# igloo-io/igloo

Hardware: AMD Instinct MI355X
Metric: TPC-H SF100 total query time (s) + rows/sec scan, 1/2/4/8 MI355X (lower is better)
Workload: dtype exact decimal(15,2) int64 fixed-point / int32 keys

## Files before the change

csrc/bindings.cpp:

```cpp
#include <pybind11/pybind11.h>
#include <pybind11/stl.h>

#include <tuple>
#include <memory>
#include <vector>

#include "io/parquet_meta.h"
#include "kernels/kernels.h"
#include "runtime/runtime.h"
#include "sql/ast.h"
#include "sql/ast_py.h"

namespace py = pybind11;
using namespace igloo;

namespace {

template <typename T>
T* P(uintptr_t p) {
  return reinterpret_cast<T*>(p);
}
hipStream_t S(uintptr_t s) { return reinterpret_cast<hipStream_t>(s); }

template <typename T>
struct py_arg {
  using type = T;
  static T get(T v) { return v; }
};
template <typename T>
struct py_arg<T*> {
  using type = uintptr_t;
  static T* get(uintptr_t v) { return reinterpret_cast<T*>(v); }
};
template <auto F>
struct raw_t;
template <typename R, typename... A, R (*F)(A...)>
struct raw_t<F> {
  R operator()(typename py_arg<A>::type... a) const { return F(py_arg<A>::get(a)...); }
};
template <auto F>
constexpr raw_t<F> raw{};

using AggDescArg = std::vector<std::tuple<int, int, uintptr_t, uintptr_t, uintptr_t, uintptr_t>>;
std::vector<kern::AggDesc> agg_descs(const AggDescArg& descs) {
  std::vector<kern::AggDesc> d;
  for (auto& t : descs)
    d.push_back({std::get<0>(t), std::get<1>(t), P<const void>(std::get<2>(t)), P<const uint8_t>(std::get<3>(t)),
                 P<void>(std::get<4>(t)), P<void>(std::get<5>(t))});
  return d;
}

py::list parse(const std::string& text) {
  py::list out;
  try {
    for (auto& st : sql::parse_sql(text)) out.append(sql::to_python(st));
  } catch (const sql::ParseError& e) {
    PyErr_SetString(PyExc_SyntaxError, e.what());
    throw py::error_already_set();
  }
  return out;
}

py::list tokenize(const std::string& text) {
  py::list out;
  static const char* names[] = {"ident", "quoted_ident", "keyword", "number", "string", "op", "end"};
  try {
    for (auto& t : sql::tokenize(text)) out.append(py::make_tuple(names[t.kind], t.text, t.pos));
  } catch (const sql::ParseError& e) {
    PyErr_SetString(PyExc_SyntaxError, e.what());
    throw py::error_already_set();
  }
  return out;
}

py::dict leaf_dict(const io::PqLeaf& l) {
  py::dict d;
  d["name"] = l.name;
  d["type"] = l.type;
  d["type_length"] = l.type_length;
  d["max_def"] = l.max_def;
  d["max_rep"] = l.max_rep;
  d["converted_type"] = l.converted_type;
  d["logical"] = l.logical;
  d["tz"] = l.tz;
  d["scale"] = l.scale;
  d["precision"] = l.precision;
  return d;
}

py::dict chunk_dict(const io::PqChunk& c) {
  py::dict d;
  d["type"] = c.type;
  d["codec"] = c.codec;
  d["num_values"] = c.num_values;
  d["start"] = c.start();
  d["length"] = c.total_compressed;
  d["uncompressed"] = c.total_uncompressed;
  d["data_page_offset"] = c.data_page_offset;
  d["dictionary_page_offset"] = c.dictionary_page_offset;
  d["encodings"] = c.encodings;
  d["external"] = c.external;
  d["null_count"] = c.stats.has_nulls ? py::object(py::int_(c.stats.null_count)) : py::object(py::none());
  d["min"] = c.stats.has_min ? py::object(py::bytes(c.stats.min)) : py::object(py::none());
  d["max"] = c.stats.has_max ? py::object(py::bytes(c.stats.max)) : py::object(py::none());
  return d;
}

py::dict page_header_dict(const io::PqPageHeader& h) {
  py::dict d;
  d["type"] = h.type;
  d["header_len"] = h.header_len;
  d["compressed"] = h.compressed;
  d["uncompressed"] = h.uncompressed;
  d["num_values"] = h.num_values;
  d["encoding"] = h.encoding;
  d["def_encoding"] = h.def_encoding;
  d["num_nulls"] = h.num_nulls;
  d["num_rows"] = h.num_rows;
  d["def_len"] = h.def_len;
  d["rep_len"] = h.rep_len;
  d["is_compressed"] = h.is_compressed;
  return d;
}

kern::PqDecodeSpec decode_spec(const py::dict& d, bool need_output = true) {
  kern::PqDecodeSpec s{};
  s.phys = d["phys"].cast<int>();
  s.type_len = d["type_len"].cast<int>();
  s.out_width = d["out_width"].cast<int>();
  s.conv = d["conv"].cast<int>();
  s.conv_k = d["conv_k"].cast<int64_t>();
  s.max_def = d["max_def"].cast<int>();
  s.out = P<void>(d["out"].cast<uintptr_t>());
  s.valid = P<uint8_t>(d["valid"].cast<uintptr_t>());
  s.scratch = P<uint32_t>(d["scratch"].cast<uintptr_t>());
  s.str_len = P<int64_t>(d["str_len"].cast<uintptr_t>());
  s.str_pos = P<int64_t>(d["str_pos"].cast<uintptr_t>());
  s.codes = P<int32_t>(d["codes"].cast<uintptr_t>());
  s.dict_len = P<int64_t>(d["dict_len"].cast<uintptr_t>());
  s.dict_pos = P<int64_t>(d["dict_pos"].cast<uintptr_t>());
  s.raw = P<const uint8_t>(d["raw"].cast<uintptr_t>());
  s.dec = P<const uint8_t>(d["dec"].cast<uintptr_t>());
  s.error = P<int>(d["error"].cast<uintptr_t>());
  if (s.max_def < 0 || s.max_def > 1 || s.phys < 0 || s.phys > kern::PQ_PHYS_FLBA || !s.raw || !s.error)
    throw std::runtime_error("pq_decode: bad spec");
  if (need_output && (s.phys == kern::PQ_PHYS_BYTE_ARRAY ? !(s.codes || (s.str_len && s.str_pos)) : !s.out))
    throw std::runtime_error("pq_decode: missing output buffer");
  return s;
}

}

namespace igloo {
void register_jit(py::module_& m);
void register_arrow_device(py::module_& m);
}

PYBIND11_MODULE(_native, m) {
  m.doc() = "igloo MI355X native core: SQL frontend, gfx950 kernels, device runtime";
  m.attr("ARCH") = "gfx950";
  m.attr("MAX_AGGS") = kern::kMaxAggs;
  m.attr("MAX_GATHER_COLS") = kern::kMaxGatherCols;
  m.attr("MAX_PARTS") = kern::kMaxParts;
  igloo::register_jit(m);
  igloo::register_arrow_device(m);

  m.def("parse_sql", &parse, "Parse SQL text into a list of statement ASTs (dicts)");
  m.def("tokenize", &tokenize);

  m.def("device_count", &rt::device_count);
  m.def("device_info", [](int dev) {
    auto d = rt::device_info(dev);
    py::dict r;
    r["device"] = d.device;
    r["name"] = d.name;
    r["arch"] = d.arch;
    r["total_mem"] = d.total_mem;
    r["free_mem"] = d.free_mem;
    r["cu_count"] = d.cu_count;
    r["wave_size"] = d.wave_size;
    r["lds_per_block"] = d.lds_per_block;
    r["l2_bytes"] = d.l2_bytes;
    r["clock_khz"] = d.clock_khz;
    return r;
  });
  py::class_<rt::PinnedPool>(m, "PinnedPool")
      .def(py::init<size_t>())
      .def("acquire",
           [](rt::PinnedPool& p, size_t bytes) {
             size_t got = 0;
             void* ptr = p.acquire(bytes, &got);
             return py::make_tuple((uintptr_t)ptr, got);
           })
      .def("release", [](rt::PinnedPool& p, uintptr_t ptr, size_t bytes) { p.release((void*)ptr, bytes); })
      .def_property_readonly("cached_bytes", &rt::PinnedPool::cached_bytes);

  m.def("select_num_tiles", &kern::select_num_tiles);
  m.def("select_count", raw<&kern::select_count>);
  m.def("select_scan_counts", [](uintptr_t counts, int64_t tiles, uintptr_t total, uintptr_t s) {
    if (!counts || !total || tiles <= 0) throw std::runtime_error("select_scan_counts: bad arguments");
    kern::scan_counts(P<int64_t>(counts), tiles, P<int64_t>(total), S(s));
  });
  m.def("select_write", raw<&kern::select_write>);
  m.def("select_compact", [](uintptr_t mask, int64_t n, uintptr_t tiles,
                             const std::vector<std::tuple<uintptr_t, uintptr_t, int, uintptr_t, uintptr_t>>& cols,
                             uintptr_t idx, bool idx64, int64_t cap, uintptr_t s) {
    kern::CompactArgs a{};
    if ((int)cols.size() > kern::kMaxCompactCols) throw std::runtime_error("select_compact: too many columns");
    for (size_t j = 0; j < cols.size(); ++j) {
      auto& c = cols[j];
      a.cols[j] = {P<void>(std::get<0>(c)), P<void>(std::get<1>(c)), std::get<2>(c), P<uint8_t>(std::get<3>(c)),
                   P<uint8_t>(std::get<4>(c))};
    }
    a.ncols = (int)cols.size();
    a.idx = P<void>(idx);
    a.idx64 = idx64;
    kern::select_compact(P<uint8_t>(mask), n, P<int64_t>(tiles), a, cap, S(s));
  });
  m.def("scan_workspace_tiles", &kern::scan_workspace_tiles);
  m.def("exclusive_scan", raw<&kern::exclusive_scan>);
  auto pack_spec = [](const std::vector<std::tuple<uintptr_t, uintptr_t, int, int>>& cols, int row_bytes) {
    if (cols.size() > (size_t)kern::kMaxPackCols) throw std::runtime_error("pack: too many columns");
    kern::PackSpec spec{};
    spec.ncols = (int32_t)cols.size();
    spec.row_bytes = row_bytes;
    for (size_t i = 0; i < cols.size(); ++i) {
      spec.cols[i].src = P<const void>(std::get<0>(cols[i]));
      spec.cols[i].dst = P<void>(std::get<1>(cols[i]));
      spec.cols[i].width = std::get<2>(cols[i]);
      spec.cols[i].offset = std::get<3>(cols[i]);
      if (spec.cols[i].offset + spec.cols[i].width > row_bytes) throw std::runtime_error("pack: field outside row");
    }
    return spec;
  };
  m.def("pack_rows", [pack_spec](std::vector<std::tuple<uintptr_t, uintptr_t, int, int>> cols, int row_bytes,
                                 uintptr_t perm, bool perm64, int64_t n, uintptr_t out, uintptr_t s) {
    kern::pack_rows(pack_spec(cols, row_bytes), P<const void>(perm), perm64, n, P<uint8_t>(out), S(s));
  });
  m.def("unpack_rows", [pack_spec](std::vector<std::tuple<uintptr_t, uintptr_t, int, int>> cols, int row_bytes,
                                   uintptr_t in, int64_t n, uintptr_t s) {
    kern::unpack_rows(pack_spec(cols, row_bytes), P<const uint8_t>(in), n, S(s));
  });
  m.def("column_stats", raw<&kern::column_stats>);
  m.def("run_bounds", raw<&kern::run_bounds>);
  m.def("mark_slot_rows", raw<&kern::mark_slot_rows>);
  m.def("pack_bits", [](std::vector<uintptr_t> cols, std::vector<bool> is64, std::vector<int64_t> lo,
                        std::vector<int> shift, int64_t n, uintptr_t out, uintptr_t s) {
    std::vector<const void*> c(cols.size());
    std::unique_ptr<bool[]> w(new bool[cols.size()]);
    for (size_t i = 0; i < cols.size(); ++i) {
      c[i] = reinterpret_cast<const void*>(cols[i]);
      w[i] = is64[i];
    }
    kern::pack_bits(c.data(), w.get(), lo.data(), shift.data(), (int)cols.size(), n, P<int64_t>(out), S(s));
  });
  m.def("differs_from_rep", raw<&kern::differs_from_rep>);
  m.def("mark_keys", raw<&kern::mark_keys>);
  m.def("probe_marks", raw<&kern::probe_marks>);
  m.def("const_ints", [](uintptr_t out, std::vector<int64_t> vals, uintptr_t s) {
    kern::const_ints(P<int64_t>(out), vals.data(), (int64_t)vals.size(), S(s));
  });
  m.def("end_capture", raw<&kern::end_capture>);
  m.def("wide_fits", raw<&kern::wide_fits>);
  m.def("avg_wide", raw<&kern::avg_wide>);
  m.def("radix_sort_ws_bytes", &kern::radix_sort_ws_bytes);
  m.def("radix_sort_pairs", raw<&kern::radix_sort_pairs>);
  m.def("sort_key_pack", [](std::vector<std::tuple<uintptr_t, uintptr_t, uint64_t, uint64_t, int, int, int, int, int>> cols,
                            uintptr_t perm, bool perm64, int64_t n, uintptr_t out, bool out32, uintptr_t s) {
    if (cols.empty() || cols.size() > (size_t)kern::kMaxSortCols) throw std::runtime_error("sort_key_pack: bad column count");
    kern::SortKeySpec spec{};
    spec.ncols = (int32_t)cols.size();
    int total = 0;
    for (size_t i = 0; i < cols.size(); ++i) {
      auto& c = spec.cols[i];
      const auto& t = cols[i];
      c.ptr = P<const void>(std::get<0>(t));
      c.valid = P<const uint8_t>(std::get<1>(t));
      c.lo = std::get<2>(t);
      c.span = std::get<3>(t);
      c.kind = std::get<4>(t);
      c.width = std::get<5>(t);
      c.bits = std::get<6>(t);
      c.desc = std::get<7>(t);
      c.nulls_first = std::get<8>(t);
      if (c.bits < 0 || c.bits > 64) throw std::runtime_error("sort_key_pack: bad field width");
      total += c.bits + (c.valid ? 1 : 0);
    }
    if (total > (out32 ? 32 : 64)) throw std::runtime_error("sort_key_pack: key fields exceed the key width");
    kern::sort_key_pack(spec, P<const void>(perm), perm64, n, P<void>(out), out32, S(s));
  });
  m.def("radix_digit_hist", raw<&kern::radix_digit_hist>);
  m.def("radix_le_mask", raw<&kern::radix_le_mask>);

  py::class_<kern::JoinTableRef>(m, "JoinTableRef")
      .def(py::init([](uintptr_t tkeys, uintptr_t thead, uintptr_t cstart, uintptr_t crows, bool rid64, int64_t cap,
                       int64_t kmin, bool direct, uintptr_t bits, uint64_t bmask, uintptr_t fold, int64_t n_build) {
             return kern::JoinTableRef{P<int64_t>(tkeys), P<void>(thead), P<void>(cstart), P<void>(crows),
                                       rid64,             cap,            kmin,            direct,
                                       P<uint32_t>(bits), bmask,          P<uint32_t>(fold), n_build};
           }),
           py::kw_only(), py::arg("tkeys"), py::arg("thead"), py::arg("cstart") = 0, py::arg("crows") = 0,
           py::arg("rid64"), py::arg("cap"), py::arg("kmin"), py::arg("direct"), py::arg("bits") = 0,
           py::arg("bmask") = 0, py::arg("fold") = 0, py::arg("n_build"));
  py::class_<kern::KeyColumn>(m, "KeyColumn")
      .def(py::init([](uintptr_t keys, bool key64, uintptr_t valid, int64_t n) {
             return kern::KeyColumn{P<const void>(keys), key64, P<const uint8_t>(valid), n};
           }),
           py::arg("keys"), py::arg("key64"), py::arg("valid"), py::arg("n"));
  m.def("join_build", raw<&kern::join_build>);
  m.def("join_csr_count", raw<&kern::join_csr_count>);
  m.def("join_csr_scatter", raw<&kern::join_csr_scatter>);
  m.def("join_probe", raw<&kern::join_probe>);
  m.def("probe_hit_tiles", &kern::probe_hit_tiles);
  m.def("probe_hits", raw<&kern::probe_hits>);
  m.def("set_probe_grid_cap", &kern::set_probe_grid_cap);
  m.def("set_probe_bits", &kern::set_probe_bits);
  m.def("set_probe_stream_min_rows", &kern::set_probe_stream_min_rows);
  m.def("set_probe_stream_max_fill", &kern::set_probe_stream_max_fill);
  m.def("last_probe_kernel", []() { return std::string(kern::last_probe_kernel()); });
  m.attr("kFoldMinRows") = kern::probe_fold_min_rows();
  m.attr("kFoldWords") = kern::probe_fold_words();
  m.def("probe_fold_needed", &kern::probe_fold_needed);
  m.def("probe_fold_build", [](uintptr_t bits, int64_t cap, uintptr_t fold, uintptr_t s) {
    if (!bits || !fold || cap <= 0) throw std::runtime_error("probe_fold_build: null buffer");
    kern::probe_fold_build(P<const uint32_t>(bits), cap, P<uint32_t>(fold), S(s));
  });
  m.def("join_table_init", [](uintptr_t thead, bool rid64, int64_t cap, uintptr_t tkeys, uintptr_t bits, int64_t nbw,
                              uintptr_t dups, uintptr_t s) {
    if (!thead || !dups || cap <= 0 || (bits && nbw <= 0)) throw std::runtime_error("join_table_init: null buffer");
    kern::join_table_init(P<void>(thead), rid64, cap, P<int64_t>(tkeys), P<uint32_t>(bits), nbw,
                          P<unsigned long long>(dups), S(s));
  });
  m.def("probe_write", raw<&kern::probe_write>);
  m.def("join_expand", raw<&kern::join_expand>);
  using FfCols = std::vector<std::pair<uintptr_t, int64_t>>;
  using FfTerms = std::vector<std::tuple<int, int, int64_t, int64_t, uint64_t>>;
  using FfKeys = std::vector<std::tuple<int, int64_t, int64_t>>;
  using FfAggs = std::vector<std::tuple<int, int, std::vector<std::tuple<int64_t, int64_t, int64_t>>, uintptr_t,
                                        uintptr_t, int, int>>;
  auto make_ff = [](const FfCols& cols, const FfTerms& terms, uintptr_t mask) {
    if (cols.size() > (size_t)kern::kFfMaxCols || terms.size() > (size_t)kern::kFfMaxTerms)
      throw std::runtime_error("fused scan: too many columns / terms");
    kern::FfSpec f{};
    f.ncols = (int32_t)cols.size();
    for (size_t i = 0; i < cols.size(); ++i) {
      f.cols[i].ptr = reinterpret_cast<const void*>(cols[i].first);
      f.cols[i].width = cols[i].second;
      const int64_t w = f.cols[i].width;
      if (!(w == 1 || w == 2 || w == 4 || w == 8) || (cols[i].first % (w < 4 ? 4 : w)) != 0)
        throw std::runtime_error("fused scan: bad column width / alignment");
    }
    f.nterms = (int32_t)terms.size();
    for (size_t i = 0; i < terms.size(); ++i) {
      auto [col, kind, lo, hi, set] = terms[i];
      const int base = kind & 0xff, grp = kind >> 8;
      if (col < 0 || col >= f.ncols || kind < 0 || base > 3 || grp > 31 || (base == 3 && (int64_t)set >= f.ncols))
        throw std::runtime_error("fused scan: bad term");
      f.terms[i] = kern::FfTerm{col, kind, lo, hi, set};
    }
    f.mask = P<const uint8_t>(mask);
    return f;
  };
  m.def("ff_mask", [make_ff](const FfCols& cols, const FfTerms& terms, uintptr_t mask, int64_t n, uintptr_t out,
                             uintptr_t s) {
    kern::FfSpec f = make_ff(cols, terms, mask);
    kern::ff_mask(f, n, P<uint8_t>(out), S(s));
  });
  m.def("ff_aggregate", [make_ff](const FfCols& cols, const FfTerms& terms, uintptr_t mask, const FfKeys& keys,
                                  int ngroups, const FfAggs& aggs, uintptr_t counts, uintptr_t overflow, int64_t n,
                                  uintptr_t s) {
    kern::FfSpec f = make_ff(cols, terms, mask);
    if (keys.size() > 2 || ngroups < 1 || ngroups > kern::kFfMaxGroups || aggs.size() > (size_t)kern::kFfMaxAggs)
      throw std::runtime_error("fused aggregate: shape out of range");
    f.nkeys = (int32_t)keys.size();
    for (size_t i = 0; i < keys.size(); ++i) {
      auto [col, lo, mul] = keys[i];
      if (col < 0 || col >= f.ncols) throw std::runtime_error("fused aggregate: bad key column");
      f.key_col[i] = col;
      f.key_lo[i] = lo;
      f.key_mul[i] = mul;
    }
    f.ngroups = ngroups;
    f.naggs = (int32_t)aggs.size();
    for (size_t i = 0; i < aggs.size(); ++i) {
      auto& [op, checked, facs, dst, dst2, shared, vbits] = aggs[i];
      if (op < 0 || op > 3 || facs.size() > (size_t)kern::kFfMaxFactors)
        throw std::runtime_error("fused aggregate: bad aggregate");
      if (shared < 0 || shared > (int)facs.size() || (shared > 0 && (i == 0 || f.aggs[i - 1].nfac != shared)))
        throw std::runtime_error("fused aggregate: bad shared prefix");
      kern::FfAgg& A = f.aggs[i];
      A.op = op;
      A.checked = checked;
      A.shared = shared;
      A.nfac = (int32_t)facs.size();
      for (size_t k = 0; k < facs.size(); ++k) {
        auto [col, a, b] = facs[k];
        if (col >= f.ncols) throw std::runtime_error("fused aggregate: bad factor column");
        A.f[k] = kern::FfFactor{col, a, b};
      }
      A.dst = P<int64_t>(dst);
      A.dst2 = P<int64_t>(dst2);
      A.vbits = vbits > 0 && vbits < 64 ? vbits : 64;
    }
    f.counts = P<int64_t>(counts);
    f.overflow = P<int>(overflow);
    kern::ff_aggregate(f, n, S(s));
  });
  m.def("ff_set_mfma", &kern::ff_set_mfma);
  m.attr("HLL_REGISTERS") = kern::kHllRegisters;
  m.def("hll_blocks", &kern::hll_blocks);
  m.def("hll_sketch", raw<&kern::hll_sketch>);
  m.def("groupby_build", raw<&kern::groupby_build>);
  m.def("groupby_occupied", raw<&kern::groupby_occupied>);
  m.def("groupby_assign", raw<&kern::groupby_assign>);
  m.def("groupby_lookup", raw<&kern::groupby_lookup>);
  m.def("fill_runs", raw<&kern::fill_runs>);

  m.def("agg_lds_max_groups", &kern::agg_lds_max_groups);
  m.def("agg_update", [](uintptr_t gid, int64_t n, int ngroups, const AggDescArg& descs, uintptr_t s,
                         bool sorted_gids) {
    auto d = agg_descs(descs);
    kern::agg_update(P<const int32_t>(gid), n, ngroups, d.data(), (int)d.size(), S(s), sorted_gids);
  }, py::arg("gid"), py::arg("n"), py::arg("ngroups"), py::arg("descs"), py::arg("s"), py::arg("sorted_gids") = false);
  m.def("agg_part_buckets", &kern::agg_part_buckets);
  m.def("agg_part_blocks", &kern::agg_part_blocks);
  m.def("agg_partitioned", [](uintptr_t gid, int64_t n, int64_t ngroups, const AggDescArg& descs, int phase,
                              uintptr_t cnt, uintptr_t off, uintptr_t total, uintptr_t pg,
                              const std::vector<uintptr_t>& vals, uintptr_t s) {
    if (!gid || n >= (int64_t(1) << 31) || ngroups <= 0 || ngroups >= (int64_t(1) << 31) || phase < 0 || phase > 2 ||
        descs.empty() || descs.size() > 8 || vals.size() != descs.size() || (phase == 0 && !cnt) ||
        (phase >= 1 && (!off || !pg)) || (phase == 2 && !total))
      throw std::runtime_error("agg_partitioned: bad arguments");
    auto d = agg_descs(descs);
    std::vector<int64_t*> v;
    for (auto x : vals) v.push_back(P<int64_t>(x));
    kern::agg_partitioned(P<const int32_t>(gid), n, ngroups, d.data(), (int)d.size(), phase, P<int32_t>(cnt),
                          P<const int64_t>(off), P<const int64_t>(total), P<uint16_t>(pg), v.data(), S(s));
  });
  m.def("sorted_having", [](uintptr_t keys, bool key64, int64_t n, const AggDescArg& descs, int hagg, int hop,
                            long long hlo, long long hhi, double hf, uintptr_t rep, int64_t cap, uintptr_t counter,
                            uintptr_t s) {
    auto d = agg_descs(descs);
    kern::sorted_having(P<const void>(keys), key64, n, d.data(), (int)d.size(), hagg, hop, hlo, hhi, hf,
                        P<int64_t>(rep), cap, P<unsigned long long>(counter), S(s));
  });
  m.def("key_histogram", [](uintptr_t keys, bool key64, uintptr_t valid, int64_t n, int64_t kmin, int64_t span,
                            uintptr_t counts, uintptr_t s) {
    if (n > 0 && (!keys || !counts || span <= 0)) throw std::runtime_error("key_histogram: bad arguments");
    kern::key_histogram(P<const void>(keys), key64, P<const uint8_t>(valid), n, kmin, span, P<int32_t>(counts), S(s));
  });
  m.def("key_histogram_buckets", &kern::key_histogram_buckets);
  m.def("key_histogram_blocks", &kern::key_histogram_blocks);
  m.def("key_histogram_partitioned", [](uintptr_t keys, bool key64, uintptr_t valid, int64_t n, int64_t kmin,
                                        int64_t span, int phase, uintptr_t cnt, uintptr_t off, int64_t total,
                                        uintptr_t part, uintptr_t counts, uintptr_t s) {
    if (span <= 0 || span > (int64_t(1) << 27) || n >= (int64_t(1) << 31) || phase < 0 || phase > 2 || !keys ||
        (phase == 0 && !cnt) || (phase >= 1 && (!off || !part)) || (phase == 2 && !counts))
      throw std::runtime_error("key_histogram_partitioned: bad arguments");
    kern::key_histogram_partitioned(P<const void>(keys), key64, P<const uint8_t>(valid), n, kmin, span, phase,
                                    P<int32_t>(cnt), P<const int64_t>(off), total, P<uint16_t>(part),
                                    P<int32_t>(counts), S(s));
  });

  m.def("gather_multi", [](uintptr_t idx, bool idx64, int64_t n, const std::vector<std::tuple<uintptr_t, uintptr_t, int, uintptr_t, uintptr_t, int64_t>>& descs, uintptr_t s) {
    std::vector<kern::GatherDesc> d;
    for (auto& t : descs)
      d.push_back({P<const void>(std::get<0>(t)), P<void>(std::get<1>(t)), std::get<2>(t),
                   P<const uint8_t>(std::get<3>(t)), P<uint8_t>(std::get<4>(t)), std::get<5>(t)});
    kern::gather_multi(P<const void>(idx), idx64, n, d.data(), (int)d.size(), S(s));
  });
  m.def("gather_packed", [](uintptr_t idx, bool idx64, int64_t n, uintptr_t src, int64_t rows, int row_bytes,
                            const std::vector<std::tuple<uintptr_t, int, int, int, int>>& fields, uintptr_t s) {
    std::vector<kern::PackedField> f;
    for (auto& t : fields)
      f.push_back({P<void>(std::get<0>(t)), std::get<1>(t), std::get<2>(t), std::get<3>(t), std::get<4>(t)});
    kern::gather_packed(P<const void>(idx), idx64, n, P<const uint8_t>(src), rows, row_bytes, f.data(), (int)f.size(),
                        S(s));
  });
  m.def("str_gather_lengths", raw<&kern::str_gather_lengths>);
  m.def("str_gather_copy", raw<&kern::str_gather_copy>);

  m.def("str_like", raw<&kern::str_like>);
  m.def("str_case", raw<&kern::str_case>);
  m.def("str_substr_lengths", raw<&kern::str_substr_lengths>);
  m.def("str_substr_copy", raw<&kern::str_substr_copy>);
  m.def("str_char_length", raw<&kern::str_char_length>);
  m.def("str_concat2_lengths", raw<&kern::str_concat2_lengths>);
  m.def("str_concat2_copy", raw<&kern::str_concat2_copy>);
  m.def("fmt_lengths", raw<&kern::fmt_lengths>);
  m.def("fmt_write", raw<&kern::fmt_write>);
  m.def("str_parse", raw<&kern::str_parse>);
  m.def("try_parse", raw<&kern::try_parse>);
  m.def("cast_checked", raw<&kern::cast_checked>);
  m.def("str_prefix_keys", raw<&kern::str_prefix_keys>);
  m.def("str_hash64", raw<&kern::str_hash64>);
  m.def("str_like_segments", raw<&kern::str_like_segments>);
  m.def("str_eq_rows", raw<&kern::str_eq_rows>);
  m.def("str_in_set", [](uintptr_t off, uintptr_t chars, int64_t n, uintptr_t vb, uintptr_t voff, uintptr_t vmode,
                         int nv, uintptr_t out, uintptr_t s) {
    if (n > 0 && (!off || !out || nv < 0 || (nv > 0 && (!vb || !voff || !vmode))))
      throw std::runtime_error("str_in_set: bad arguments");
    kern::str_in_set(P<const int64_t>(off), P<const uint8_t>(chars), n, P<const uint8_t>(vb), P<const int32_t>(voff),
                     P<const uint8_t>(vmode), nv, P<uint8_t>(out), S(s));
  });
  m.def("str_cmp_const", raw<&kern::str_cmp_const>);
  m.def("str_prefix_key", raw<&kern::str_prefix_key>);

  m.attr("CSV_TILE") = kern::kCsvTile;
  m.attr("CSV_COLUMN_BYTES") = (int)sizeof(kern::CsvColumn);
  m.def("csv_num_tiles", &kern::csv_num_tiles);
  m.def("csv_quote_parity", [](uintptr_t buf, int64_t n, int quote, uintptr_t tile_par, uintptr_t s) {
    kern::csv_quote_parity(P<const uint8_t>(buf), n, (uint8_t)quote, P<uint8_t>(tile_par), S(s));
  });
  m.def("csv_rows", [](uintptr_t buf, int64_t n, int64_t start, int quote, uintptr_t tile_state, uintptr_t tile_rows,
                       uintptr_t tile_off, uintptr_t rows_end, uintptr_t s) {
    kern::csv_rows(P<const uint8_t>(buf), n, start, (uint8_t)quote, P<const uint8_t>(tile_state),
                   P<int64_t>(tile_rows), P<const int64_t>(tile_off), P<int64_t>(rows_end), S(s));
  });
  m.def("csv_pack_columns", [](const std::vector<std::tuple<int, int, uintptr_t, uintptr_t, uintptr_t>>& cols) {
    std::vector<kern::CsvColumn> v;
    for (auto& [kind, scale, out, len, valid] : cols) {
      if (kind < kern::CSV_SKIP || kind > kern::CSV_UTF8) throw std::runtime_error("csv: bad column kind");
      if (kind != kern::CSV_SKIP && !out) throw std::runtime_error("csv: missing output buffer");
      if (kind == kern::CSV_UTF8 && !len) throw std::runtime_error("csv: missing length buffer");
      v.push_back({kind, scale, P<void>(out), P<int64_t>(len), P<uint8_t>(valid)});
    }
    return py::bytes(reinterpret_cast<const char*>(v.data()), v.size() * sizeof(kern::CsvColumn));
  });
  m.def("csv_parse", [](uintptr_t buf, int64_t start, uintptr_t rows_end, int64_t nrows, uintptr_t cols, int ncols,
                        int delim, int quote, uintptr_t err, uintptr_t s) {
    kern::csv_parse(P<const uint8_t>(buf), start, P<const int64_t>(rows_end), nrows,
                    P<const kern::CsvColumn>(cols), ncols, (uint8_t)delim, (uint8_t)quote, P<int>(err), S(s));
  });
  m.def("csv_str_lengths", raw<&kern::csv_str_lengths>);
  m.def("csv_str_copy", [](uintptr_t pos, uintptr_t len_flag, uintptr_t off, int64_t n, int quote, uintptr_t out,
                           uintptr_t s) {
    kern::csv_str_copy(P<const int64_t>(pos), P<const int64_t>(len_flag), P<const int64_t>(off), n, (uint8_t)quote,
                       P<uint8_t>(out), S(s));
  });

  m.def("strfmt_lengths", [](const std::string& fmt, bool is_date, uintptr_t v, uintptr_t offs, int64_t n,
                             uintptr_t len, uintptr_t s) {
    kern::strfmt_lengths(reinterpret_cast<const uint8_t*>(fmt.data()), (int)fmt.size(), is_date, P<const void>(v),
                         P<const int32_t>(offs), n, P<int64_t>(len), S(s));
  });
  m.def("strfmt_write", [](const std::string& fmt, bool is_date, uintptr_t v, uintptr_t offs, int64_t n,
                           uintptr_t off, int64_t out_cap, uintptr_t out, uintptr_t s) {
    kern::strfmt_write(reinterpret_cast<const uint8_t*>(fmt.data()), (int)fmt.size(), is_date, P<const void>(v),
                       P<const int32_t>(offs), n, P<const int64_t>(off), out_cap, P<uint8_t>(out), S(s));
  });
  m.def("tz_to_local", raw<&kern::tz_to_local>);
  m.def("tz_to_utc", raw<&kern::tz_to_utc>);
  m.def("tz_trunc", raw<&kern::tz_trunc>);
  m.def("tz_part", raw<&kern::tz_part>);
  m.def("regex_lds_bytes", &kern::regex_lds_bytes);
  m.def("regex_dfa_match", raw<&kern::regex_dfa_match>);
  using SpanDfaArg = std::tuple<uintptr_t, uintptr_t, uintptr_t, int, int, bool, bool>;
  auto span_dfa = [](const SpanDfaArg& d) {
    return kern::RegexSpanDfa{P<const uint16_t>(std::get<0>(d)), P<const uint8_t>(std::get<1>(d)),
                              P<const uint8_t>(std::get<2>(d)), std::get<3>(d), std::get<4>(d), std::get<5>(d),
                              std::get<6>(d)};
  };
  m.def("regex_span_count", [span_dfa](const SpanDfaArg& d, uintptr_t off, uintptr_t chars, int64_t n, bool all,
                                       int64_t repl_len, int64_t start_char, uintptr_t out, uintptr_t exhausted,
                                       uintptr_t s) {
    kern::regex_span_count(span_dfa(d), P<const int64_t>(off), P<const uint8_t>(chars), n, all, repl_len, start_char,
                           P<int64_t>(out), P<int64_t>(exhausted), S(s));
  });
  m.def("regex_span_first", [span_dfa](const SpanDfaArg& d, uintptr_t off, uintptr_t chars, int64_t n,
                                       uintptr_t out_pos, uintptr_t out_len, uintptr_t exhausted, uintptr_t s) {
    kern::regex_span_first(span_dfa(d), P<const int64_t>(off), P<const uint8_t>(chars), n, P<int64_t>(out_pos),
                           P<int64_t>(out_len), P<int64_t>(exhausted), S(s));
  });
  m.def("regex_span_replace", [span_dfa](const SpanDfaArg& d, uintptr_t off, uintptr_t chars, int64_t n, bool all,
                                         uintptr_t repl, int64_t repl_len, uintptr_t new_off, uintptr_t out,
                                         int64_t cap, uintptr_t s) {
    kern::regex_span_replace(span_dfa(d), P<const int64_t>(off), P<const uint8_t>(chars), n, all,
                             P<const uint8_t>(repl), repl_len, P<const int64_t>(new_off), P<uint8_t>(out), cap, S(s));
  });
  m.def("probe_hash16", raw<&kern::probe_hash16>);
  m.def("probe_inlist16", [](bool mfma, uintptr_t off, uintptr_t chars, int64_t n, const std::string& pats, int npat,
                             int len, uintptr_t out, uintptr_t s) {
    if ((int64_t)pats.size() < 16 * npat) throw std::runtime_error("probe_inlist16: 16 bytes per pattern");
    kern::probe_inlist16(mfma, P<const int64_t>(off), P<const uint8_t>(chars), n,
                         reinterpret_cast<const uint8_t*>(pats.data()), npat, len, P<uint8_t>(out), S(s));
  });
  m.def("digest_width", &kern::digest_width);
  m.def("digest_hex", raw<&kern::digest_hex>);
  m.def("bin_hex_encode", raw<&kern::bin_hex_encode>);
  m.def("bin_hex_validate", raw<&kern::bin_hex_validate>);
  m.def("bin_hex_decode", raw<&kern::bin_hex_decode>);
  m.def("bin_b64_enc_lengths", raw<&kern::bin_b64_enc_lengths>);
  m.def("bin_b64_dec_lengths", raw<&kern::bin_b64_dec_lengths>);
  m.def("bin_b64_write", raw<&kern::bin_b64_write>);
  m.def("utf8_num_tiles", &kern::utf8_num_tiles);
  m.def("utf8_validate", raw<&kern::utf8_validate>);
  m.def("uuid_v4", raw<&kern::uuid_v4>);
  m.def("list_element_idx", raw<&kern::list_element_idx>);
  m.def("interleave_idx", raw<&kern::interleave_idx>);
  m.def("list_slots", raw<&kern::list_slots>);
  m.attr("LIST_FAST_MAX") = (int)kern::kListFastMax;
  m.def("map_lookup_idx", raw<&kern::map_lookup_idx>);
  m.def("map_lookup_idx_str", raw<&kern::map_lookup_idx_str>);
  m.def("list_slice_se", raw<&kern::list_slice_se>);
  m.def("list_parts_count", raw<&kern::list_parts_count>);
  m.def("list_parts_write", raw<&kern::list_parts_write>);
  m.def("list_flatten_count", raw<&kern::list_flatten_count>);
  m.def("list_flatten_write", raw<&kern::list_flatten_write>);
  m.def("list_match_count", raw<&kern::list_match_count>);
  m.def("list_match_write", raw<&kern::list_match_write>);
  m.def("list_minmax_idx", raw<&kern::list_minmax_idx>);
  m.def("list_set_count", raw<&kern::list_set_count>);
  m.def("list_set_write", raw<&kern::list_set_write>);
  m.def("list_sort_idx", raw<&kern::list_sort_idx>);
  m.def("json_parse", [](uintptr_t buf, int64_t start, uintptr_t rows_end, int64_t nrows, uintptr_t cols, int ncols,
                         uintptr_t names, uintptr_t name_off, uintptr_t err, uintptr_t s) {
    if (ncols > 64) throw std::runtime_error("json_parse: at most 64 fields");
    kern::json_parse(P<const uint8_t>(buf), start, P<const int64_t>(rows_end), nrows, P<const kern::CsvColumn>(cols),
                     ncols, P<const uint8_t>(names), P<const int32_t>(name_off), P<int>(err), S(s));
  });
  m.def("json_str_copy", raw<&kern::json_str_copy>);

  m.def("sorted_ranges", raw<&kern::sorted_ranges>);
  m.attr("SEARCH_FENCE") = kern::kFence;
  m.attr("STATS_SLOTS") = kern::kStatsSlots;
  m.def("expand_ranges", raw<&kern::expand_ranges>);

  m.def("dense_index_build", [](uintptr_t big, bool key64, int64_t nb, int64_t kmin, int64_t kmax, uintptr_t first,
                                bool first64, uintptr_t long_gap, uintptr_t s) {
    if (nb <= 0 || kmax < kmin || !big || !first) throw std::runtime_error("dense_index_build: bad arguments");
    kern::dense_index_build(P<const void>(big), key64, nb, kmin, kmax, P<void>(first), first64, P<int32_t>(long_gap),
                            S(s));
  });
  m.def("dense_ranges", [](uintptr_t first, bool first64, int64_t kmin, int64_t kmax, uintptr_t q, bool key64,
                           uintptr_t qvalid, int64_t nq, uintptr_t lo, uintptr_t cnt, uintptr_t s) {
    if (nq > 0 && (!first || !q || !lo || !cnt)) throw std::runtime_error("dense_ranges: null buffer");
    kern::dense_ranges(P<const void>(first), first64, kmin, kmax, P<const void>(q), key64, P<const uint8_t>(qvalid), nq,
                       P<int64_t>(lo), P<int64_t>(cnt), S(s));
  });
  m.def("unique_lookup", [](uintptr_t big, bool key64, int64_t nb, uintptr_t first, bool first64, int64_t kmin,
                            int64_t kmax, uintptr_t q, uintptr_t qvalid, int64_t nq, uintptr_t hit, uintptr_t pos,
                            uintptr_t fence, int64_t nf, uintptr_t s) {
    if (nq > 0 && (!q || !hit || !pos || (!first && !big))) throw std::runtime_error("unique_lookup: null buffer");
    if (nb >= (int64_t{1} << 31)) throw std::runtime_error("unique_lookup: positions must fit int32");
    kern::unique_lookup(P<const void>(big), key64, nb, P<const void>(first), first64, kmin, kmax, P<const void>(q),
                        P<const uint8_t>(qvalid), nq, P<uint8_t>(hit), P<int32_t>(pos), P<const void>(fence), nf,
                        S(s));
  });
  m.def("sorted_exists", [](uintptr_t big2, uintptr_t small2, bool key64, uintptr_t lo, uintptr_t cnt, int64_t ns,
                            int op, uintptr_t mask, uintptr_t hit, uintptr_t s) {
    if (op < 0 || op > 6 || (op == 6 && !mask) || (ns > 0 && (!lo || !cnt || !hit || (op < 6 && (!big2 || !small2)))))
      throw std::runtime_error("sorted_exists: bad arguments");
    kern::sorted_exists(P<const void>(big2), P<const void>(small2), key64, P<const int64_t>(lo), P<const int64_t>(cnt),
                        ns, op, P<const uint8_t>(mask), P<uint8_t>(hit), S(s));
  });
  m.def("sorted_match", [](uintptr_t big2, uintptr_t small2, bool key64, uintptr_t lo, uintptr_t cnt, int64_t ns,
                           uintptr_t counts, uintptr_t offsets, uintptr_t sidx, uintptr_t bidx, bool out64,
                           int64_t out_cap, uintptr_t first, uintptr_t s) {
    if (ns > 0 && (!big2 || !small2 || !lo || !cnt || (!offsets && !counts) || (offsets && (!sidx || !bidx))))
      throw std::runtime_error("sorted_match: null buffer");
    kern::sorted_match(P<const void>(big2), P<const void>(small2), key64, P<const int64_t>(lo), P<const int64_t>(cnt),
                       ns, P<int32_t>(counts), P<const int64_t>(offsets), P<void>(sidx), P<void>(bidx), out64,
                       out_cap, P<int32_t>(first), S(s));
  });
  m.def("sorted_masked", [](uintptr_t mask, uintptr_t lo, uintptr_t cnt, int64_t ns, uintptr_t counts,
                            uintptr_t offsets, uintptr_t sidx, uintptr_t bidx, bool out64, int64_t out_cap,
                            uintptr_t s) {
    if (ns > 0 && (!mask || !lo || !cnt || (!offsets && !counts) || (offsets && (!sidx || !bidx))))
      throw std::runtime_error("sorted_masked: null buffer");
    kern::sorted_masked(P<const uint8_t>(mask), P<const int64_t>(lo), P<const int64_t>(cnt), ns, P<int32_t>(counts),
                        P<const int64_t>(offsets), P<void>(sidx), P<void>(bidx), out64, out_cap, S(s));
  });

  m.def("partition_run_blocks", &kern::partition_run_blocks);
  m.def("partition_run", raw<&kern::partition_run>);
  m.def("partition_ids", raw<&kern::partition_ids>);
  m.def("date_part", raw<&kern::date_part>);
  m.def("str_fn_lengths", [](int fn, int64_t n1, uintptr_t a, int64_t alen, uintptr_t b, int64_t blen, uintptr_t off,
                             uintptr_t chars, int64_t n, uintptr_t len, uintptr_t s) {
    kern::StrFnArgs args{fn, n1, P<uint8_t>(a), alen, P<uint8_t>(b), blen};
    kern::str_fn_lengths(args, P<int64_t>(off), P<uint8_t>(chars), n, P<int64_t>(len), S(s));
  });
  m.def("str_fn_copy", [](int fn, int64_t n1, uintptr_t a, int64_t alen, uintptr_t b, int64_t blen, uintptr_t off,
                          uintptr_t chars, int64_t n, uintptr_t new_off, uintptr_t out, int64_t out_cap,
                          uintptr_t s) {
    kern::StrFnArgs args{fn, n1, P<uint8_t>(a), alen, P<uint8_t>(b), blen};
    kern::str_fn_copy(args, P<int64_t>(off), P<uint8_t>(chars), n, P<int64_t>(new_off), P<uint8_t>(out), out_cap,
                      S(s));
  });
  m.def("str_fn_int", raw<&kern::str_fn_int>);
  m.attr("LEV_FAST_MAX") = (int)kern::kLevFastMax;
  m.def("str_pair_int", raw<&kern::str_pair_int>);
  m.def("str_levenshtein", raw<&kern::str_levenshtein>);
  m.def("str_levenshtein_long", raw<&kern::str_levenshtein_long>);
  m.def("win_scan_tiles", &kern::win_scan_tiles);
  m.def("win_seg_scan", raw<&kern::win_seg_scan>);
  m.def("win_bounds", raw<&kern::win_bounds>);
  m.def("win_frame_sum", raw<&kern::win_frame_sum>);
  m.def("win_sparse_build", raw<&kern::win_sparse_build>);
  m.def("win_sparse_query", raw<&kern::win_sparse_query>);
  m.def("win_frame_minmax", raw<&kern::win_frame_minmax>);
  m.def("win_rank", raw<&kern::win_rank>);
  m.def("win_index", raw<&kern::win_index>);

  m.def("pq_file_meta", [](const std::string& path) {
    io::PqFileMeta meta;
    {
      py::gil_scoped_release rel;
      meta = io::read_file_meta(path);
    }
    py::dict d;
    d["version"] = meta.version;
    d["num_rows"] = meta.num_rows;
    d["created_by"] = meta.created_by;
    py::list leaves, groups;
    for (auto& l : meta.leaves) leaves.append(leaf_dict(l));
    for (auto& g : meta.row_groups) {
      py::dict gd;
      gd["num_rows"] = g.num_rows;
      py::list cs;
      for (auto& c : g.chunks) cs.append(chunk_dict(c));
      gd["chunks"] = cs;
      groups.append(gd);
    }
    d["leaves"] = leaves;
    d["row_groups"] = groups;
    return d;
  }, "Parse a Parquet footer (native Thrift compact decoder)");
  m.def("pq_page_headers", [](uintptr_t host, int64_t n) {
    py::list out;
    for (auto& h : io::parse_chunk_pages(P<const uint8_t>(host), (size_t)n)) out.append(page_header_dict(h));
    return out;
  });
  m.def("pq_pread", [](const std::string& path, const std::vector<std::tuple<int64_t, int64_t, uintptr_t>>& ranges,
                       int threads) {
    std::vector<io::ReadRange> rs;
    for (auto& [off, len, dst] : ranges) {
      if (off < 0 || len < 0 || !dst) throw std::runtime_error("pq_pread: bad range");
      rs.push_back({off, len, P<uint8_t>(dst)});
    }
    py::gil_scoped_release rel;
    io::pread_ranges(path, rs, threads);
  });
  m.def("pq_plan", [](uintptr_t host, const std::vector<std::tuple<int64_t, int64_t, int, int64_t, int64_t>>& chunks,
                      int phys, int max_def, int max_rep, int64_t dec_base, int type_len) {
    std::vector<io::PqChunkIn> cs;
    for (auto& [off, len, codec, first, rows] : chunks) cs.push_back({off, len, codec, first, rows});
    io::PqPlan plan;
    {
      py::gil_scoped_release rel;
      plan = io::plan_column(P<const uint8_t>(host), cs, phys, max_def, max_rep, dec_base, type_len);
    }
    py::dict d;
    d["pages"] = py::bytes((const char*)plan.pages.data(), plan.pages.size());
    d["jobs"] = py::bytes((const char*)plan.jobs.data(), plan.jobs.size());
    d["num_pages"] = plan.num_pages;
    d["num_jobs"] = plan.num_jobs;
    d["num_zstd_jobs"] = plan.num_zstd_jobs;
    d["num_dict_pages"] = plan.num_dict_pages;
    d["dec_bytes"] = plan.dec_bytes;
    d["dict_entries"] = plan.dict_entries;
    d["plain_pages"] = plan.plain_pages;
    d["max_page_values"] = plan.max_page_values;
    d["unsupported"] = plan.unsupported;
    return d;
  }, "Plan GPU decode descriptors for one column's chunks staged at `host`",
     py::arg("host"), py::arg("chunks"), py::arg("phys"), py::arg("max_def"), py::arg("max_rep"),
     py::arg("dec_base") = 0, py::arg("type_len") = 0);
  m.def("pq_pack_spec", [](const py::dict& spec, bool need_output) {
    kern::PqDecodeSpec sp = decode_spec(spec, need_output);
    return py::bytes(reinterpret_cast<const char*>(&sp), sizeof(sp));
  }, "Validated binary PqDecodeSpec (concatenate one per column and upload)");
  m.attr("PQ_SPEC_BYTES") = (int)sizeof(kern::PqDecodeSpec);
  m.def("pq_zstd_slots", &kern::pq_zstd_slots);
  m.def("pq_zstd", [](uintptr_t jobs, int64_t njobs, uintptr_t raw, uintptr_t dec, uintptr_t lit, int64_t slots,
                      uintptr_t err, uintptr_t s) {
    if (njobs > 0 && (!jobs || !raw || !dec || !lit || !err)) throw std::runtime_error("pq_zstd: null buffer");
    kern::pq_zstd(P<const kern::PqSnappyJob>(jobs), njobs, P<const uint8_t>(raw), P<uint8_t>(dec), P<uint8_t>(lit),
                  slots, P<int>(err), S(s));
  });
  m.def("zstd_decompress_host", [](py::bytes src, int64_t size) {
    std::string in = src;
    std::string out((size_t)size, '\0');
    int e;
    {
      py::gil_scoped_release nogil;
      e = kern::zstd_decompress_host((const uint8_t*)in.data(), (int64_t)in.size(), (uint8_t*)out.data(), size);
    }
    return py::make_tuple(e, py::bytes(out));
  });
  m.def("pq_snappy", [](uintptr_t jobs, int64_t njobs, uintptr_t raw, uintptr_t dec, uintptr_t err, uintptr_t s) {
    if (njobs > 0 && (!jobs || !raw || !dec || !err)) throw std::runtime_error("pq_snappy: null buffer");
    kern::pq_snappy(P<const kern::PqSnappyJob>(jobs), njobs, P<const uint8_t>(raw), P<uint8_t>(dec), P<int>(err), S(s));
  });
  m.def("pq_dict_strings", [](uintptr_t pages, int64_t npages, uintptr_t page_col, uintptr_t specs, uintptr_t s) {
    if (npages > 0 && (!pages || !page_col || !specs)) throw std::runtime_error("pq_dict_strings: null buffer");
    kern::pq_dict_strings(P<const kern::PqPage>(pages), npages, P<const int32_t>(page_col),
                          P<const kern::PqDecodeSpec>(specs), S(s));
  });
  m.def("pq_decode", [](uintptr_t pages, int64_t npages, uintptr_t page_col, uintptr_t specs, uintptr_t s) {
    if (npages > 0 && (!pages || !page_col || !specs)) throw std::runtime_error("pq_decode: null buffer");
    kern::pq_decode(P<const kern::PqPage>(pages), npages, P<const int32_t>(page_col),
                    P<const kern::PqDecodeSpec>(specs), S(s));
  });
  m.def("pq_str_copy", raw<&kern::pq_str_copy>);

  auto mkparams = [](const py::tuple& t) {
    kern::TextGenParams p;
    p.kind = t[0].cast<int>();
    p.seed = t[1].cast<uint64_t>();
    p.row_base = t[2].cast<int64_t>();
    p.min_len = t[3].cast<int>();
    p.max_len = t[4].cast<int>();
    p.vocab = P<const uint8_t>(t[5].cast<uintptr_t>());
    p.vocab_off = P<const int32_t>(t[6].cast<uintptr_t>());
    p.vocab_n = t[7].cast<int>();
    p.inject = P<const uint8_t>(t[8].cast<uintptr_t>());
    p.inject_len = t[9].cast<int>();
    p.inject_every = t[10].cast<int>();
    p.suffix_char = t[11].cast<int>();
    p.aux = P<const int32_t>(t[12].cast<uintptr_t>());
    p.row_ids = t.size() > 13 ? P<const int64_t>(t[13].cast<uintptr_t>()) : nullptr;
    return p;
  };
  m.def("textgen_lengths", [mkparams](const py::tuple& t, int64_t n, uintptr_t lens, bool device, uintptr_t s) {
    auto p = mkparams(t);
    py::gil_scoped_release rel;
    kern::textgen_lengths(p, n, P<int64_t>(lens), device, S(s));
  });
  m.def("textgen_write", [mkparams](const py::tuple& t, int64_t n, uintptr_t off, uintptr_t chars, bool device, uintptr_t s) {
    auto p = mkparams(t);
    py::gil_scoped_release rel;
    kern::textgen_write(p, n, P<const int64_t>(off), P<uint8_t>(chars), device, S(s));
  });
}
```

csrc/kernels/kernels.h:

```cpp
#pragma once

#include <hip/hip_runtime.h>

#include <cstdint>

namespace igloo {
namespace kern {

constexpr int kMaxAggs = 8;
constexpr int kMaxGatherCols = 16;
constexpr int kMaxParts = 64;

int64_t select_num_tiles(int64_t n);
void select_count(const uint8_t* mask, int64_t n, int64_t* tile_counts, int64_t* total, hipStream_t stream);
void select_write(const uint8_t* mask, int64_t n, const int64_t* tile_offsets, void* out, bool idx64, int64_t cap,
                  hipStream_t stream);
void scan_counts(int64_t* counts, int64_t n, int64_t* total, hipStream_t stream);
constexpr int kMaxCompactCols = 12;
struct CompactCol {
  const void* src;
  void* dst;
  int esz;
  const uint8_t* sv;
  uint8_t* dv;
};
struct CompactArgs {
  CompactCol cols[kMaxCompactCols];
  int ncols;
  void* idx;
  bool idx64;
};
void select_compact(const uint8_t* mask, int64_t n, const int64_t* tile_offsets, const CompactArgs& a, int64_t cap,
                    hipStream_t stream);
int64_t scan_workspace_tiles(int64_t n);
void exclusive_scan(const void* in, bool in64, int64_t n, int64_t* out, int64_t* tile_ws, int64_t* total,
                    hipStream_t stream);

constexpr int kMaxSortCols = 8;
struct SortKeyCol {
  const void* ptr;
  const uint8_t* valid;
  uint64_t lo, span;
  int32_t kind, width, bits, desc, nulls_first, pad;
};
struct SortKeySpec {
  int32_t ncols, pad;
  SortKeyCol cols[kMaxSortCols];
};
int64_t radix_sort_ws_bytes(int64_t n);
int radix_sort_pairs(void* k0, void* k1, bool key64, void* v0, void* v1, bool val64, int64_t n, int begin_bit,
                     int end_bit, void* ws, hipStream_t stream);
void sort_key_pack(const SortKeySpec& spec, const void* perm, bool perm64, int64_t n, void* out, bool out32,
                   hipStream_t stream);
void radix_digit_hist(const void* keys, bool key64, int64_t n, int shift, uint64_t prefix, int pshift,
                      unsigned long long* hist, hipStream_t stream);
void radix_le_mask(const void* keys, bool key64, int64_t n, uint64_t bound, uint8_t* mask, hipStream_t stream);

constexpr int kMaxPackCols = 48;
struct PackCol {
  const void* src;
  void* dst;
  int32_t width, offset;
};
struct PackSpec {
  int32_t ncols, row_bytes;
  PackCol cols[kMaxPackCols];
};
void pack_rows(const PackSpec& spec, const void* perm, bool perm64, int64_t n, uint8_t* out, hipStream_t stream);
void unpack_rows(const PackSpec& spec, const uint8_t* in, int64_t n, hipStream_t stream);

void const_ints(int64_t* out, const int64_t* vals, int64_t n, hipStream_t stream);
constexpr int kMaxPackBits = 8;
void pack_bits(const void* const* cols, const bool* is64, const int64_t* lo, const int* shift, int ncols, int64_t n,
               int64_t* out, hipStream_t stream);
void differs_from_rep(const void* a, int elem_bytes, const void* rep, bool rep64, int64_t n, int* flag,
                      hipStream_t stream);
void mark_slot_rows(const int32_t* trow, int64_t cap, int64_t n, uint8_t* mark, hipStream_t stream);
void mark_keys(const void* keys, bool key64, const uint8_t* valid, int64_t n, int64_t kmin, int64_t dom,
               uint8_t* marks, hipStream_t stream);
void probe_marks(const void* keys, bool key64, const uint8_t* valid, int64_t n, int64_t base, int64_t dom,
                 const uint8_t* marks, bool negate, uint8_t* out, hipStream_t stream);
void end_capture(hipStream_t stream);
constexpr int kStatsMaxBlocks = 4096;
constexpr int kStatsSlots = 3 + 3 * kStatsMaxBlocks;
void column_stats(const void* keys, bool key64, const uint8_t* valid, int64_t n, long long* out, hipStream_t stream);
void run_bounds(const void* keys, bool key64, int64_t n, uint8_t* out, hipStream_t stream);

constexpr int kFfMaxCols = 8;
constexpr int kFfMaxTerms = 16;
constexpr int kFfMaxAggs = 8;
constexpr int kFfMaxGroups = 16;
constexpr int kFfMaxFactors = 3;
struct FfColumn {
  const void* ptr;
  int64_t width;
};
struct FfTerm {
  int32_t col, kind;
  int64_t lo, hi;
  uint64_t set;
};
struct FfFactor {
  int64_t col, a, b;
};
struct FfAgg {
  int32_t op, nfac;
  int32_t checked, shared;
  FfFactor f[kFfMaxFactors];
  int64_t* dst;
  int64_t* dst2;
  int32_t vbits, pad;
};
struct FfSpec {
  int32_t ncols, nterms, nkeys, naggs, ngroups, pad;
  FfColumn cols[kFfMaxCols];
  FfTerm terms[kFfMaxTerms];
  int32_t key_col[2];
  int64_t key_lo[2];
  int64_t key_mul[2];
  FfAgg aggs[kFfMaxAggs];
  const uint8_t* mask;
  int64_t* counts;
  int* overflow;
};
void ff_mask(const FfSpec& spec, int64_t n, uint8_t* out, hipStream_t stream);
void ff_aggregate(const FfSpec& spec, int64_t n, hipStream_t stream);
bool ff_set_mfma(bool on);

constexpr int kHllBits = 12;
constexpr int kHllRegisters = 1 << kHllBits;
constexpr int kHllMaxBlocks = 1024;
int hll_blocks(int64_t n);
void hll_sketch(const void* keys, bool key64, const uint8_t* valid, int64_t n, uint8_t* block_regs, uint8_t* regs,
                hipStream_t stream);

struct JoinTableRef {
  int64_t* tkeys;
  void* thead;
  void* cstart;
  void* crows;
  bool rid64;
  int64_t cap, kmin;
  bool direct;
  uint32_t* bits;
  uint64_t bmask;
  uint32_t* fold;
  int64_t n_build;
};
struct KeyColumn {
  const void* keys;
  bool key64;
  const uint8_t* valid;
  int64_t n;
};
void check(const JoinTableRef& t, const char* what);
void join_build(const JoinTableRef& t, const KeyColumn& build, unsigned long long* dups, hipStream_t stream);
void join_csr_count(const JoinTableRef& t, const KeyColumn& build, void* cnt, hipStream_t stream);
void join_csr_scatter(const JoinTableRef& t, const KeyColumn& build, void* cnt, hipStream_t stream);
void join_probe(const JoinTableRef& t, const KeyColumn& probe, bool use_filter, int32_t* counts, void* first,
                uint8_t* build_matched, hipStream_t stream);
int64_t probe_hit_tiles(int64_t m);
void set_probe_grid_cap(int cap);
void set_probe_bits(int mode);
void set_probe_stream_min_rows(int64_t rows);
void set_probe_stream_max_fill(double fill);
int64_t probe_fold_min_rows();
int probe_fold_words();
const char* last_probe_kernel();
bool probe_fold_needed(int64_t m, int64_t cap);
void probe_fold_build(const uint32_t* bits, int64_t cap, uint32_t* fold, hipStream_t stream);
void probe_hits(const JoinTableRef& t, const KeyColumn& probe, bool use_filter, bool negate,
                unsigned long long* words, int64_t* tile_counts, hipStream_t stream);
void join_table_init(void* thead, bool rid64, int64_t cap, int64_t* tkeys, uint32_t* bits, int64_t nbw,
                     unsigned long long* dups, hipStream_t stream);
void probe_write(const JoinTableRef& t, const KeyColumn& probe, const unsigned long long* words,
                 const int64_t* tile_off, void* out_probe, bool out64, void* out_build, int64_t out_cap,
                 hipStream_t stream);
void join_expand(const JoinTableRef& t, const KeyColumn& probe, bool use_filter, const int64_t* offsets,
                 int32_t* out_probe, void* out_build, int64_t out_cap, hipStream_t stream);
void fill_runs(const void* starts, bool starts64, int64_t nruns, int64_t n, int32_t* gid, hipStream_t stream);
void groupby_build(const void* keys, bool key64, int64_t n, int64_t* tkeys, int32_t* trow, int64_t cap, int64_t kmin,
                   bool direct, hipStream_t stream);
void groupby_occupied(const int32_t* trow, int64_t cap, uint8_t* occ, int32_t* gid_of_slot, hipStream_t stream);
void groupby_assign(const void* slots, bool slots64, int64_t g, int64_t cap, const int32_t* trow,
                    int32_t* gid_of_slot, int32_t* rep_row, hipStream_t stream);
void groupby_lookup(const void* keys, bool key64, int64_t n, const int64_t* tkeys, const int32_t* gid_of_slot,
                    int64_t cap, int64_t kmin, bool direct, int32_t* gid, hipStream_t stream);

enum AggOp : int {
  AGG_SUM_INT = 0,
  AGG_SUM_F64 = 1,
  AGG_COUNT = 2,
  AGG_MIN_INT = 3,
  AGG_MAX_INT = 4,
  AGG_MIN_F64 = 5,
  AGG_MAX_F64 = 6,
  AGG_BIT_AND = 7,
  AGG_BIT_OR = 8,
  AGG_BIT_XOR = 9,
};

struct AggDesc {
  int op;
  int src64;
  const void* src;
  const uint8_t* valid;
  void* dst;
  void* dst2;
  int64_t groups = 0;
};

int agg_lds_max_groups(int nagg);
void sorted_having(const void* keys, bool key64, int64_t n, const AggDesc* descs, int nagg, int hagg, int hop,
                   long long hlo, long long hhi, double hf, int64_t* rep, int64_t cap, unsigned long long* counter,
                   hipStream_t stream);
void key_histogram(const void* keys, bool key64, const uint8_t* valid, int64_t n, int64_t kmin, int64_t span,
                   int32_t* counts, hipStream_t stream);
int key_histogram_buckets(int64_t span);
int key_histogram_blocks();
void key_histogram_partitioned(const void* keys, bool key64, const uint8_t* valid, int64_t n, int64_t kmin,
                               int64_t span, int phase, int32_t* cnt, const int64_t* off, int64_t total,
                               uint16_t* part, int32_t* counts, hipStream_t stream);
int agg_part_bits(int nagg);
int agg_part_buckets(int64_t ngroups, int nagg);
int agg_part_blocks();
void agg_partitioned(const int32_t* gid, int64_t n, int64_t ngroups, const AggDesc* descs, int nagg, int phase,
                     int32_t* cnt, const int64_t* off, const int64_t* total, uint16_t* pg, int64_t* const* vals,
                     hipStream_t stream);
void agg_update(const int32_t* gid, int64_t n, int ngroups, const AggDesc* descs, int nagg, hipStream_t stream,
                bool sorted_gids = false);

struct GatherDesc {
  const void* src;
  void* dst;
  int elem_bytes;
  const uint8_t* src_valid;
  uint8_t* dst_valid;
  int64_t src_rows;
};
void gather_multi(const void* idx, bool idx64, int64_t n, const GatherDesc* descs, int ncols, hipStream_t stream);
constexpr int kMaxPackedFields = 16;
constexpr int kPackedSigned = 1;
constexpr int kPackedInRange = 2;
struct PackedField {
  void* dst;
  int32_t off;
  int32_t width;
  int32_t out_bytes;
  int32_t flags;
};
void gather_packed(const void* idx, bool idx64, int64_t n, const uint8_t* src, int64_t src_rows, int row_bytes,
                   const PackedField* fields, int nf, hipStream_t stream);
void str_gather_lengths(const int64_t* off, int64_t src_rows, const void* idx, bool idx64, int64_t n, int64_t* len,
                        hipStream_t stream);
void str_gather_copy(const int64_t* off, int64_t src_rows, const uint8_t* chars, const void* idx, bool idx64,
                     int64_t n, const int64_t* new_off, uint8_t* out, int64_t out_cap, hipStream_t stream);

void str_like(const int64_t* off, const uint8_t* chars, int64_t n, const uint8_t* pat, const uint8_t* kind, int m,
              bool case_insensitive, bool negate, uint8_t* out, hipStream_t stream);
void str_case(const uint8_t* in, int64_t nbytes, bool to_upper, uint8_t* out, int* non_ascii, hipStream_t stream);
void str_substr_lengths(const int64_t* off, const uint8_t* chars, int64_t n, int64_t start, int64_t len, bool has_len,
                        int64_t* out_len, hipStream_t stream);
void str_substr_copy(const int64_t* off, const uint8_t* chars, int64_t n, int64_t start, int64_t len, bool has_len,
                     const int64_t* new_off, uint8_t* out, hipStream_t stream);
void str_char_length(const int64_t* off, const uint8_t* chars, int64_t n, int32_t* out, hipStream_t stream);
void str_concat2_lengths(const int64_t* oa, bool ba, const int64_t* ob, bool bb, int64_t n, int64_t* len,
                         hipStream_t stream);
void str_concat2_copy(const int64_t* oa, const uint8_t* ca, bool ba, const int64_t* ob, const uint8_t* cb, bool bb,
                      int64_t n, const int64_t* off, uint8_t* out, hipStream_t stream);
void fmt_lengths(const void* vals, int kind, int64_t n, int scale, const uint8_t* valid, int64_t* len,
                 hipStream_t stream);
void fmt_write(const void* vals, int kind, int64_t n, int scale, const uint8_t* valid, const int64_t* off,
               uint8_t* out, hipStream_t stream);
void str_parse(const int64_t* off, const uint8_t* chars, int64_t n, const uint8_t* valid, int kind, int scale,
               void* out, int* err, hipStream_t stream);
void try_parse(const int64_t* off, const uint8_t* chars, int64_t n, const uint8_t* valid, int kind, int scale,
               int precision, void* out, uint8_t* valid_out, hipStream_t stream);
void cast_checked(const void* src, int src_kind, int src_scale, int64_t n, const uint8_t* valid_in, int dst_kind,
                  int dst_scale, int dst_precision, void* dst, uint8_t* valid_out, hipStream_t stream);
void str_like_segments(const int64_t* off, const uint8_t* chars, int64_t n, const uint8_t* seg, const int32_t* seg_off,
                       int nseg, bool anchor_start, bool anchor_end, bool negate, uint8_t* out, int64_t nbytes,
                       int min_seg, hipStream_t stream);
void wide_fits(const int64_t* lo, const int64_t* hi, int64_t n, int* flag, hipStream_t stream);
void avg_wide(const int64_t* sums, bool wide, const int64_t* cnt, int64_t n, int64_t up, int64_t* out,
              hipStream_t stream);
void str_prefix_keys(const int64_t* off, const uint8_t* chars, int64_t n, int chunks, int64_t* out,
                     hipStream_t stream);
void str_hash64(const int64_t* off, const uint8_t* chars, int64_t n, const uint8_t* valid, int64_t* out,
                hipStream_t stream);
void str_eq_rows(const int64_t* aoff, const uint8_t* achars, const void* ai, const int64_t* boff, const uint8_t* bchars,
                 const void* bi, bool idx64, int64_t n, int* mismatches, hipStream_t stream);
void str_cmp_const(const int64_t* off, const uint8_t* chars, int64_t n, const uint8_t* c, int64_t cn, int op,
                   uint8_t* out, hipStream_t stream);
void str_in_set(const int64_t* off, const uint8_t* chars, int64_t n, const uint8_t* vb, const int32_t* voff,
                const uint8_t* vmode, int nv, uint8_t* out, hipStream_t stream);
void str_prefix_key(const int64_t* off, const uint8_t* chars, int64_t n, int64_t skip, int64_t* out,
                    hipStream_t stream);

int64_t partition_run_blocks(int64_t n);
void partition_run(const void* keys, bool key64, int64_t n, int nparts, int64_t* counts_ws, int64_t* total,
                   void* perm, bool perm64, hipStream_t stream);
void partition_ids(const void* keys, bool key64, int64_t n, int nparts, int32_t* out, hipStream_t stream);
void date_part(const int32_t* days, int64_t n, int field, int32_t* out, hipStream_t stream);

enum TextKind : int {
  TEXT_WORDS = 0,
  TEXT_DISTINCT_WORDS = 1,
  TEXT_ALNUM = 2,
  TEXT_PREFIX_INT = 3,
  TEXT_PREFIX_RANDINT = 4,
  TEXT_PHONE = 5,
};

struct TextGenParams {
  int kind;
  uint64_t seed;
  int64_t row_base;
  int min_len, max_len;
  const uint8_t* vocab;
  const int32_t* vocab_off;
  int vocab_n;
  const uint8_t* inject;
  int inject_len;
  int inject_every;
  int suffix_char;
  const int32_t* aux;
  const int64_t* row_ids;
};
void textgen_lengths(const TextGenParams& p, int64_t n, int64_t* lens, bool device, hipStream_t stream);
void textgen_write(const TextGenParams& p, int64_t n, const int64_t* off, uint8_t* chars, bool device,
                   hipStream_t stream);

constexpr int64_t kCsvTile = 16 * 1024;
enum CsvKind : int { CSV_SKIP = 0, CSV_INT32 = 1, CSV_INT64 = 2, CSV_DECIMAL = 3, CSV_FLOAT64 = 4, CSV_DATE = 5,
                     CSV_BOOL = 6, CSV_UTF8 = 7 };
struct CsvColumn {
  int32_t kind, scale;
  void* out;
  int64_t* len;
  uint8_t* valid;
};
int64_t csv_num_tiles(int64_t n);
void csv_quote_parity(const uint8_t* buf, int64_t n, uint8_t quote, uint8_t* tile_par, hipStream_t stream);
void csv_rows(const uint8_t* buf, int64_t n, int64_t start, uint8_t quote, const uint8_t* tile_state,
              int64_t* tile_rows, const int64_t* tile_off, int64_t* rows_end, hipStream_t stream);
void csv_parse(const uint8_t* buf, int64_t start, const int64_t* rows_end, int64_t nrows, const CsvColumn* cols,
               int ncols, uint8_t delim, uint8_t quote, int* err, hipStream_t stream);
void csv_str_lengths(const int64_t* len_flag, int64_t n, int64_t* len, hipStream_t stream);
void csv_str_copy(const int64_t* pos, const int64_t* len_flag, const int64_t* off, int64_t n, uint8_t quote,
                  uint8_t* out, hipStream_t stream);

enum DigestAlgo : int { kDigestMd5 = 0, kDigestSha224 = 1, kDigestSha256 = 2, kDigestSha384 = 3, kDigestSha512 = 4,
                        kDigestBlake2b = 5, kDigestBlake2s = 6 };
int digest_width(int algo);
void digest_hex(int algo, const int64_t* off, const uint8_t* chars, int64_t n, uint8_t* out, hipStream_t s);
void uuid_v4(uint64_t seed, int64_t n, uint8_t* out, hipStream_t s);

void strfmt_lengths(const uint8_t* fmt, int flen, bool is_date, const void* v, const int32_t* offs, int64_t n,
                    int64_t* len, hipStream_t s);
void strfmt_write(const uint8_t* fmt, int flen, bool is_date, const void* v, const int32_t* offs, int64_t n,
                  const int64_t* off, int64_t out_cap, uint8_t* out, hipStream_t s);

void tz_to_local(const int64_t* in, int64_t n, const int64_t* tab, int log2p, int fixed_off, int64_t utc_lo,
                 int64_t wall_lo, int64_t* out, int32_t* off_out, hipStream_t s);
void tz_to_utc(const int64_t* in, int64_t n, const int64_t* tab, int log2p, int fixed_off, int64_t utc_lo,
               int64_t wall_lo, int64_t* out, hipStream_t s);
void tz_trunc(const int64_t* in, int64_t n, const int64_t* tab, int log2p, int fixed_off, int64_t utc_lo,
              int64_t wall_lo, int unit, int64_t* out, hipStream_t s);
void tz_part(const int64_t* in, int64_t n, const int64_t* tab, int log2p, int fixed_off, int64_t utc_lo,
             int64_t wall_lo, int field, int32_t* out, hipStream_t s);

size_t regex_lds_bytes(int nstates, int nclasses);
void regex_dfa_match(const int64_t* off, const uint8_t* chars, int64_t n, const uint16_t* table, const uint8_t* cls,
                     const uint8_t* flags, int nstates, int nclasses, int start, bool anchored_end, bool negate,
                     uint8_t* out, hipStream_t s);
struct RegexSpanDfa {
  const uint16_t* table;
  const uint8_t* cls;
  const uint8_t* flags;
  int nstates, nclasses;
  bool anchored_start, anchored_end;
};
void regex_span_count(const RegexSpanDfa& d, const int64_t* off, const uint8_t* chars, int64_t n, bool all,
                      int64_t repl_len, int64_t start_char, int64_t* out, int64_t* exhausted, hipStream_t s);
void regex_span_first(const RegexSpanDfa& d, const int64_t* off, const uint8_t* chars, int64_t n, int64_t* out_pos,
                      int64_t* out_len, int64_t* exhausted, hipStream_t s);
void regex_span_replace(const RegexSpanDfa& d, const int64_t* off, const uint8_t* chars, int64_t n, bool all,
                        const uint8_t* repl, int64_t repl_len, const int64_t* new_off, uint8_t* out, int64_t cap,
                        hipStream_t s);

void probe_hash16(bool mfma, const int32_t* k0, const int32_t* k1, const int32_t* k2, const int32_t* k3, int64_t n,
                  const int8_t* proj, uint32_t* out, hipStream_t s);
void probe_inlist16(bool mfma, const int64_t* off, const uint8_t* chars, int64_t n, const uint8_t* pats, int npat,
                    int len, uint8_t* out, hipStream_t s);

void list_element_idx(const int64_t* se, const uint8_t* valid, const int64_t* pos, const uint8_t* pos_valid,
                      int64_t pos_const, int64_t n, int64_t child_n, int64_t* out, hipStream_t s);
void interleave_idx(int64_t n, int k, int64_t* out, hipStream_t s);
void list_slots(int64_t n, int64_t k, int64_t* se, hipStream_t s);
void map_lookup_idx(const int64_t* se, const uint8_t* valid, int64_t n, int64_t child_n, int key_width,
                    const void* keys, const uint8_t* kvalid, const int64_t* needle, const uint8_t* needle_valid,
                    int64_t needle_const, int64_t* out, hipStream_t s);
void map_lookup_idx_str(const int64_t* se, const uint8_t* valid, int64_t n, int64_t child_n, const int64_t* key_offs,
                        const uint8_t* key_bytes, int64_t key_nbytes, const uint8_t* kvalid,
                        const int64_t* needle_offs, const uint8_t* needle_bytes, int64_t needle_nbytes,
                        const uint8_t* needle_valid, int64_t const_len, int64_t const_stride, int64_t* out,
                        hipStream_t s);
constexpr int kListFastMax = 512;
void list_slice_se(const int64_t* se, const uint8_t* valid, const int64_t* from, const uint8_t* from_valid,
                   const int64_t* to, const uint8_t* to_valid, int64_t from_const, int64_t to_const, int64_t n,
                   int64_t* out_se, uint8_t* out_valid, hipStream_t s);
void list_parts_count(const int64_t* parts, int k, int64_t n, int64_t* out_len, hipStream_t s);
void list_parts_write(const int64_t* parts, int k, int64_t n, const int64_t* offs, int64_t src_n, int64_t cap,
                      int64_t* idx, int64_t* out_se, hipStream_t s);
void list_flatten_count(const int64_t* se, const uint8_t* valid, const int64_t* ise, const uint8_t* ivalid,
                        int64_t n, int64_t inner_n, int64_t* out_len, hipStream_t s);
void list_flatten_write(const int64_t* se, const uint8_t* valid, const int64_t* ise, const uint8_t* ivalid,
                        int64_t n, int64_t inner_n, const int64_t* offs, int64_t child_n, int64_t cap,
                        int64_t* idx, int64_t* out_se, hipStream_t s);
void list_match_count(const int64_t* se, const uint8_t* valid, const int64_t* keys, const uint8_t* kvalid,
                      int64_t child_n, const int64_t* needle, const uint8_t* needle_valid, const int64_t* from,
                      const int64_t* limit, int64_t limit_const, int mode, int64_t n, int64_t* out, hipStream_t s);
void list_match_write(const int64_t* se, const uint8_t* valid, const int64_t* keys, const uint8_t* kvalid,
                      int64_t child_n, const int64_t* needle, const uint8_t* needle_valid, const int64_t* limit,
                      int64_t limit_const, int mode, int64_t n, const int64_t* offs, int64_t repl_base,
                      int64_t cap, int64_t* out, hipStream_t s);
void list_minmax_idx(const int64_t* se, const uint8_t* valid, const int64_t* keys, const uint8_t* kvalid,
                     int64_t child_n, int is_max, int64_t n, int64_t* out, hipStream_t s);
void list_set_count(const int64_t* seA, const uint8_t* validA, const int64_t* keysA, const uint8_t* kvalidA,
                    int64_t childA_n, const int64_t* seB, const uint8_t* validB, const int64_t* keysB,
                    const uint8_t* kvalidB, int64_t childB_n, int op, int64_t n, int64_t* out, hipStream_t s);
void list_set_write(const int64_t* seA, const uint8_t* validA, const int64_t* keysA, const uint8_t* kvalidA,
                    int64_t childA_n, const int64_t* seB, const uint8_t* validB, const int64_t* keysB,
                    const uint8_t* kvalidB, int64_t childB_n, int op, int64_t n, const int64_t* offs,
                    int64_t b_base, int64_t cap, int64_t* idx, hipStream_t s);
void list_sort_idx(const int64_t* se, const uint8_t* valid, const int64_t* keys, const uint8_t* kvalid,
                   int64_t child_n, int desc, int nulls_first, int64_t n, const int64_t* offs, int64_t cap,
                   int64_t* idx, hipStream_t s);

void json_parse(const uint8_t* buf, int64_t start, const int64_t* rows_end, int64_t nrows, const CsvColumn* cols,
                int ncols, const uint8_t* names, const int32_t* name_off, int* err, hipStream_t stream);
void json_str_copy(const int64_t* pos, const int64_t* len_flag, const int64_t* off, int64_t n, uint8_t* out,
                   hipStream_t stream);

constexpr int64_t kFence = 256;
void sorted_ranges(const void* big, bool key64, int64_t nb, const void* q, const uint8_t* qvalid, int64_t nq,
                   int64_t* lo, int64_t* cnt, const void* fence, int64_t nf, hipStream_t stream);
void expand_ranges(const int64_t* off, const int64_t* lo, int64_t ns, int64_t total, void* sidx, void* bidx,
                   bool out64, hipStream_t stream);
void dense_index_build(const void* big, bool key64, int64_t nb, int64_t kmin, int64_t kmax, void* first, bool first64,
                       int32_t* long_gap, hipStream_t stream);
void dense_ranges(const void* first, bool first64, int64_t kmin, int64_t kmax, const void* q, bool key64,
                  const uint8_t* qvalid, int64_t nq, int64_t* lo, int64_t* cnt, hipStream_t stream);
void unique_lookup(const void* big, bool key64, int64_t nb, const void* first, bool first64, int64_t kmin,
                   int64_t kmax, const void* q, const uint8_t* qvalid, int64_t nq, uint8_t* hit, int32_t* pos,
                   const void* fence, int64_t nf, hipStream_t stream);
void sorted_exists(const void* big2, const void* small2, bool key64, const int64_t* lo, const int64_t* cnt,
                   int64_t ns, int op, const uint8_t* mask, uint8_t* hit, hipStream_t stream);
void sorted_match(const void* big2, const void* small2, bool key64, const int64_t* lo, const int64_t* cnt,
                  int64_t ns, int32_t* counts, const int64_t* offsets, void* sidx, void* bidx, bool out64,
                  int64_t out_cap, int32_t* first, hipStream_t stream);
void sorted_masked(const uint8_t* mask, const int64_t* lo, const int64_t* cnt, int64_t ns, int32_t* counts,
                   const int64_t* offsets, void* sidx, void* bidx, bool out64, int64_t out_cap, hipStream_t stream);

enum PqPhys : int { PQ_PHYS_BOOLEAN = 0, PQ_PHYS_INT32 = 1, PQ_PHYS_INT64 = 2, PQ_PHYS_INT96 = 3, PQ_PHYS_FLOAT = 4,
                    PQ_PHYS_DOUBLE = 5, PQ_PHYS_BYTE_ARRAY = 6, PQ_PHYS_FLBA = 7 };
enum PqPageKind : int { PQ_PAGE_DATA_V1 = 0, PQ_PAGE_DATA_V2 = 1, PQ_PAGE_DICT = 2 };
enum PqPageFlags : int { PQ_DATA_IN_DEC = 1, PQ_DICT_IN_DEC = 2 };
enum PqConv : int { PQ_CONV_COPY = 0, PQ_CONV_NARROW = 1, PQ_CONV_SEXT = 2, PQ_CONV_ZEXT = 3, PQ_CONV_F2D = 4,
                    PQ_CONV_FLBA = 5, PQ_CONV_MUL = 6, PQ_CONV_DIV = 7, PQ_CONV_BOOL = 8 };

struct PqPage {
  int64_t data_off;
  int64_t levels_off;
  int64_t dict_off;
  int64_t out_row;
  int64_t aux_off;
  int32_t size;
  int32_t num_values;
  int32_t levels_len;
  int32_t encoding;
  int32_t kind;
  int32_t flags;
  int32_t dict_base;
  int32_t dict_count;
};
static_assert(sizeof(PqPage) == 72, "PqPage layout is shared with the host planner");

enum PqJobCodec : int { PQ_CODEC_SNAPPY = 1, PQ_CODEC_ZSTD = 6 };
struct PqSnappyJob {
  int64_t src_off;
  int64_t dst_off;
  int32_t src_len, dst_len;
  int32_t codec;
  int32_t pad;
};
static_assert(sizeof(PqSnappyJob) == 32, "PqSnappyJob layout is shared with the host planner");

struct PqDecodeSpec {
  int32_t phys, type_len, out_width, conv;
  int64_t conv_k;
  int32_t max_def, pad;
  void* out;
  uint8_t* valid;
  uint32_t* scratch;
  int64_t* str_len;
  int64_t* str_pos;
  int32_t* codes;
  int64_t* dict_len;
  int64_t* dict_pos;
  const uint8_t* raw;
  const uint8_t* dec;
  int* error;
};

void pq_snappy(const PqSnappyJob* jobs, int64_t njobs, const uint8_t* raw, uint8_t* dec, int* error,
               hipStream_t stream);
constexpr int64_t kZstdMaxSlots = 1024;
int64_t pq_zstd_slots(int64_t njobs);
void pq_zstd(const PqSnappyJob* jobs, int64_t njobs, const uint8_t* raw, uint8_t* dec, uint8_t* lit, int64_t slots,
             int* error, hipStream_t stream);
int zstd_decompress_host(const uint8_t* src, int64_t slen, uint8_t* dst, int64_t dcap);
void pq_dict_strings(const PqPage* pages, int64_t npages, const int32_t* page_col, const PqDecodeSpec* specs,
                     hipStream_t stream);
void pq_decode(const PqPage* pages, int64_t npages, const int32_t* page_col, const PqDecodeSpec* specs,
               hipStream_t stream);
void pq_str_copy(const int64_t* pos, const int64_t* off, int64_t n, uint8_t* out, hipStream_t stream);

enum WinVal { kWinI64 = 0, kWinI32 = 1, kWinF64 = 2, kWinOne = 3, kWinHeadIdx = 4, kWinHead2 = 5 };
enum WinFn {
  kWinRowNumber = 0, kWinRank = 1, kWinDenseRank = 2, kWinPercentRank = 3, kWinCumeDist = 4, kWinNtile = 5,
  kWinLag = 10, kWinFirst = 11, kWinLast = 12, kWinNth = 13
};
int64_t win_scan_tiles(int64_t n);
void win_seg_scan(const void* ids, bool ids64, const void* ids2, bool ids2_64, const void* vals, int vkind,
                  const uint8_t* valid, int64_t n, int op, bool reverse, int* tflag, int64_t* tval, int64_t* out,
                  int* err, hipStream_t s);
void win_bounds(int64_t n, const int64_t* seg_start, const int64_t* seg_end, const int64_t* peer_start,
                const int64_t* peer_end, int unit, int skind, int64_t soff_i, double soff_f, int ekind,
                int64_t eoff_i, double eoff_f, const void* key, bool key_f64, const uint8_t* key_valid, bool desc,
                const int64_t* gnum, const int64_t* gpos, int64_t ngroups, int64_t* lo, int64_t* hi,
                hipStream_t s);
void win_frame_sum(const int64_t* psum, bool f64, const int64_t* pcnt, const int64_t* lo, const int64_t* hi,
                   int64_t n, int64_t* sum_out, int64_t* cnt_out, hipStream_t s);
void win_sparse_build(const int64_t* vals, bool f64, const uint8_t* valid, int64_t n, bool is_max, int levels,
                      int64_t* table, hipStream_t s);
void win_sparse_query(const int64_t* table, int levels, int64_t n, const int64_t* lo, const int64_t* hi,
                      const int64_t* pcnt, bool is_max, bool f64, int64_t* out, uint8_t* out_valid, hipStream_t s);
void win_frame_minmax(const int64_t* vals, bool f64, bool is_max, const uint8_t* valid, const int64_t* lo,
                      const int64_t* hi, int64_t n, int64_t* out, uint8_t* out_valid, hipStream_t s);
void win_rank(int fn, int64_t arg, int64_t n, const int64_t* seg_start, const int64_t* seg_end,
              const int64_t* peer_start, const int64_t* peer_end, const int64_t* dense, int64_t* out,
              hipStream_t s);
void win_index(int fn, int64_t arg, int64_t n, const int64_t* seg_start, const int64_t* seg_end, const int64_t* lo,
               const int64_t* hi, int64_t* out, hipStream_t s);

enum StrFnCode {
  kSfTrim = 0, kSfReplace = 1, kSfLpad = 2, kSfRpad = 3, kSfReverse = 4, kSfRepeat = 5, kSfLeft = 6, kSfRight = 7,
  kSfInitcap = 8, kSfTranslate = 9, kSfSplitPart = 10, kSfSubstrIndex = 11,
  kSfStrpos = 20, kSfAscii = 21, kSfOctetLength = 22
};
struct StrFnArgs {
  int fn;
  int64_t n1;
  const uint8_t* a;
  int64_t alen;
  const uint8_t* b;
  int64_t blen;
};
void str_fn_lengths(const StrFnArgs& a, const int64_t* off, const uint8_t* chars, int64_t n, int64_t* len,
                    hipStream_t s);
void str_fn_copy(const StrFnArgs& a, const int64_t* off, const uint8_t* chars, int64_t n, const int64_t* new_off,
                 uint8_t* out, int64_t out_cap, hipStream_t s);
void str_fn_int(int fn, const uint8_t* pat, int64_t plen, const int64_t* off, const uint8_t* chars, int64_t n,
                int32_t* out, hipStream_t s);

enum StrPairCode { kSpStrpos = 0, kSpContains = 1, kSpStartsWith = 2, kSpEndsWith = 3, kSpFindInSet = 4 };
constexpr int kLevFastMax = 127;
void str_pair_int(int fn, const int64_t* oa, const uint8_t* ca, bool ba, const int64_t* ob, const uint8_t* cb, bool bb,
                  int64_t n, int32_t* out, hipStream_t s);
void str_levenshtein(const int64_t* oa, const uint8_t* ca, bool ba, const int64_t* ob, const uint8_t* cb, bool bb,
                     int64_t n, int32_t* out, int64_t* left, hipStream_t s);
void str_levenshtein_long(const int64_t* oa, const uint8_t* ca, bool ba, const int64_t* ob, const uint8_t* cb, bool bb,
                          int64_t n, int32_t* out, int32_t* scratch, int64_t lanes, int64_t cells, hipStream_t s);

void bin_hex_encode(const uint8_t* in, int64_t nbytes, uint8_t* out, hipStream_t s);
void bin_hex_validate(const int64_t* off, const uint8_t* chars, const uint8_t* valid, int64_t n, int64_t nbytes,
                      int64_t* err, hipStream_t s);
void bin_hex_decode(const int64_t* off, int64_t n, const uint8_t* in, int64_t nout, uint8_t* out, hipStream_t s);
void bin_b64_enc_lengths(const int64_t* off, const uint8_t* valid, int64_t n, int64_t* lens, hipStream_t s);
void bin_b64_dec_lengths(const int64_t* off, const uint8_t* chars, const uint8_t* valid, int64_t n, int64_t nbytes,
                         int64_t* lens, int64_t* err, hipStream_t s);
void bin_b64_write(bool encode, const int64_t* ioff, const uint8_t* chars, const int64_t* ooff, int64_t n,
                   int64_t out_cap, uint8_t* out, hipStream_t s);
int64_t utf8_num_tiles(int64_t nbytes);
void utf8_validate(const int64_t* off, const uint8_t* chars, const uint8_t* valid, int64_t n, int64_t nbytes,
                   uint8_t* flags, int64_t* err, hipStream_t s);

}
}
```

csrc/kernels/ranges.hip:

```cpp
#include "common.h"
#include "kernels.h"
#include "launch.h"

namespace igloo {
namespace kern {

namespace {

constexpr int kExpItems = 8;
constexpr int kExpTile = kBlock * kExpItems;
constexpr int kScanRun = 16;

template <typename K>
__global__ __launch_bounds__(kBlock) void sorted_ranges_kernel(const K* __restrict__ big, int64_t nb,
                                                              const K* __restrict__ q,
                                                              const uint8_t* __restrict__ qvalid, int64_t nq,
                                                              int64_t* __restrict__ lo_out,
                                                              int64_t* __restrict__ cnt_out,
                                                              const K* __restrict__ fence, int64_t nf) {
  for (int64_t i = blockIdx.x * (int64_t)blockDim.x + threadIdx.x; i < nq; i += (int64_t)gridDim.x * blockDim.x) {
    if (qvalid && !qvalid[i]) {
      lo_out[i] = 0;
      cnt_out[i] = 0;
      continue;
    }
    const K key = q[i];
    int64_t a = 0, b = nb;
    if (fence) {
      int64_t fa = 0, fb = nf;
      while (fa < fb) {
        const int64_t m = (fa + fb) >> 1;
        if (fence[m] < key) fa = m + 1;
        else fb = m;
      }
      a = fa > 0 ? (fa - 1) * kFence : 0;
      b = fa * kFence < nb ? fa * kFence : nb;
    }
    while (a < b) {
      const int64_t m = (a + b) >> 1;
      if (big[m] < key) a = m + 1;
      else b = m;
    }
    int64_t e = a;
    int k = 0;
    while (e < nb && k < kScanRun && big[e] == key) {
      ++e;
      ++k;
    }
    if (k == kScanRun && e < nb && big[e] == key) {
      int64_t a2 = e, b2 = nb;
      while (a2 < b2) {
        const int64_t m = (a2 + b2) >> 1;
        if (big[m] <= key) a2 = m + 1;
        else b2 = m;
      }
      e = a2;
    }
    lo_out[i] = a;
    cnt_out[i] = e - a;
  }
}

__device__ inline int64_t row_of(const int64_t* off, int64_t n, int64_t t) {
  int64_t a = 0, b = n - 1;
  while (a < b) {
    const int64_t m = (a + b + 1) >> 1;
    if (off[m] <= t) a = m;
    else b = m - 1;
  }
  return a;
}

template <typename O>
__global__ __launch_bounds__(kBlock) void expand_ranges_kernel(const int64_t* __restrict__ off,
                                                              const int64_t* __restrict__ lo, int64_t ns,
                                                              int64_t total, O* __restrict__ sidx,
                                                              O* __restrict__ bidx) {
  __shared__ int64_t soff[kExpTile + 1];
  __shared__ int64_t rr[2];
  const int64_t t0 = (int64_t)blockIdx.x * kExpTile;
  if (t0 >= total) return;
  const int64_t t1 = t0 + kExpTile < total ? t0 + kExpTile : total;
  if (threadIdx.x == 0) {
    rr[0] = row_of(off, ns, t0);
    rr[1] = row_of(off, ns, t1 - 1);
  }
  __syncthreads();
  const int64_t r0 = rr[0], nr = rr[1] - rr[0] + 1;
  if (nr <= kExpTile) {
    for (int64_t k = threadIdx.x; k < nr; k += blockDim.x) soff[k] = off[r0 + k];
    __syncthreads();
    const int64_t ta = t0 + (int64_t)threadIdx.x * kExpItems;
    if (ta < t1) {
      int64_t j = row_of(soff, nr, ta);
      int64_t base = lo[r0 + j] - soff[j];
      O sv[kExpItems], bv[kExpItems];
#pragma unroll
      for (int k = 0; k < kExpItems; ++k) {
        const int64_t t = ta + k;
        while (j + 1 < nr && soff[j + 1] <= t) {
          ++j;
          base = lo[r0 + j] - soff[j];
        }
        sv[k] = (O)(r0 + j);
        bv[k] = (O)(base + t);
      }
      if (ta + kExpItems <= t1 && (((uintptr_t)(sidx + ta) | (uintptr_t)(bidx + ta)) & 15) == 0) {
        constexpr int kV = 16 / (int)sizeof(O);
        typedef O OV __attribute__((ext_vector_type(kV)));
#pragma unroll
        for (int k = 0; k < kExpItems; k += kV) {
          OV a, b;
#pragma unroll
          for (int q = 0; q < kV; ++q) {
            a[q] = sv[k + q];
            b[q] = bv[k + q];
          }
          *(OV*)(sidx + ta + k) = a;
          *(OV*)(bidx + ta + k) = b;
        }
      } else {
#pragma unroll
        for (int k = 0; k < kExpItems; ++k)
          if (ta + k < t1) {
            sidx[ta + k] = sv[k];
            bidx[ta + k] = bv[k];
          }
      }
    }
  } else {
    for (int k = 0; k < kExpItems; ++k) {
      const int64_t t = t0 + threadIdx.x + (int64_t)k * kBlock;
      if (t >= t1) break;
      const int64_t r = row_of(off, ns, t);
      sidx[t] = (O)r;
      bidx[t] = (O)(lo[r] + (t - off[r]));
    }
  }
}

}

void sorted_ranges(const void* big, bool key64, int64_t nb, const void* q, const uint8_t* qvalid, int64_t nq,
                   int64_t* lo, int64_t* cnt, const void* fence, int64_t nf, hipStream_t stream) {
  if (nq <= 0) return;
  const unsigned grid = grid_for(nq, kBlock, 1 << 16);
  dispatch(wide{key64}, [&](auto k) {
    using K = type_of<decltype(k)>;
    launch("sorted_ranges", sorted_ranges_kernel<K>, dim3(grid), dim3(kBlock), 0, stream, as<K>(big), nb, as<K>(q),
           qvalid, nq, lo, cnt, as<K>(fence), nf);
  });
}

void expand_ranges(const int64_t* off, const int64_t* lo, int64_t ns, int64_t total, void* sidx, void* bidx,
                   bool out64, hipStream_t stream) {
  if (total <= 0 || ns <= 0) return;
  const unsigned grid = (unsigned)((total + kExpTile - 1) / kExpTile);
  dispatch(wide{out64}, [&](auto o) {
    using O = type_of<decltype(o)>;
    launch("expand_ranges", expand_ranges_kernel<O>, dim3(grid), dim3(kBlock), 0, stream, off, lo, ns, total,
           as<O>(sidx), as<O>(bidx));
  });
}

}
}

namespace igloo {
namespace kern {
namespace {

template <typename K2, typename O, bool WRITE, bool MASKED = false>
__global__ __launch_bounds__(kBlock) void sorted_match_kernel(const K2* __restrict__ big2,
                                                             const K2* __restrict__ small2,
                                                             const int64_t* __restrict__ lo,
                                                             const int64_t* __restrict__ cnt, int64_t ns,
                                                             int32_t* __restrict__ counts,
                                                             const int64_t* __restrict__ offsets,
                                                             O* __restrict__ sidx, O* __restrict__ bidx,
                                                             int64_t out_cap, O* __restrict__ first) {
  const uint8_t* __restrict__ mask = reinterpret_cast<const uint8_t*>(big2);
  for (int64_t i = blockIdx.x * (int64_t)blockDim.x + threadIdx.x; i < ns; i += (int64_t)gridDim.x * blockDim.x) {
    const int64_t l = lo[i], c = cnt[i];
    const K2 key = MASKED ? K2{} : small2[i];
    int64_t o = WRITE ? offsets[i] : 0;
    int32_t m = 0;
    int64_t f = -1;
    for (int64_t k = 0; k < c; ++k) {
      if (MASKED ? mask[l + k] != 0 : big2[l + k] == key) {
        if (WRITE) {
          if (o >= 0 && o < out_cap) {
            sidx[o] = (O)i;
            bidx[o] = (O)(l + k);
          }
          ++o;
        }
        if (m == 0) f = l + k;
        ++m;
      }
    }
    if (!WRITE) {
      counts[i] = m;
      if (first) first[i] = (O)f;
    }
  }
}

template <typename K2, bool MASKED>
void launch_match(const char* what, const void* big2, const void* small2, const int64_t* lo, const int64_t* cnt,
                  int64_t ns, int32_t* counts, const int64_t* offsets, void* sidx, void* bidx, bool out64,
                  int64_t out_cap, int32_t* first, hipStream_t stream) {
  const dim3 g(grid_for(ns, kBlock, 1 << 16)), b(kBlock);
  if (!offsets) {
    launch(what, sorted_match_kernel<K2, int32_t, false, MASKED>, g, b, 0, stream, as<K2>(big2), as<K2>(small2), lo,
           cnt, ns, counts, nullptr, nullptr, nullptr, 0, first);
    return;
  }
  dispatch(wide{out64}, [&](auto o) {
    using O = type_of<decltype(o)>;
    launch(what, sorted_match_kernel<K2, O, true, MASKED>, g, b, 0, stream, as<K2>(big2), as<K2>(small2), lo, cnt, ns,
           nullptr, offsets, as<O>(sidx), as<O>(bidx), out_cap, nullptr);
  });
}

}

void sorted_match(const void* big2, const void* small2, bool key64, const int64_t* lo, const int64_t* cnt,
                  int64_t ns, int32_t* counts, const int64_t* offsets, void* sidx, void* bidx, bool out64,
                  int64_t out_cap, int32_t* first, hipStream_t stream) {
  if (ns <= 0) return;
  dispatch(wide{key64}, [&](auto k) {
    launch_match<type_of<decltype(k)>, false>("sorted_match", big2, small2, lo, cnt, ns, counts, offsets, sidx, bidx,
                                              out64, out_cap, first, stream);
  });
}

void sorted_masked(const uint8_t* mask, const int64_t* lo, const int64_t* cnt, int64_t ns, int32_t* counts,
                   const int64_t* offsets, void* sidx, void* bidx, bool out64, int64_t out_cap, hipStream_t stream) {
  if (ns <= 0) return;
  launch_match<int32_t, true>("sorted_masked", mask, nullptr, lo, cnt, ns, counts, offsets, sidx, bidx, out64, out_cap,
                              nullptr, stream);
}

}
}

namespace igloo {
namespace kern {
namespace {

constexpr int64_t kGapFill = 64;

template <typename K, typename I>
__global__ __launch_bounds__(kBlock) void dense_index_kernel(const K* __restrict__ big, int64_t nb, int64_t kmin,
                                                            int64_t kmax, I* __restrict__ first,
                                                            int32_t* __restrict__ long_gap) {
  for (int64_t i = blockIdx.x * (int64_t)blockDim.x + threadIdx.x; i <= nb; i += (int64_t)gridDim.x * blockDim.x) {
    const int64_t prev = i == 0 ? kmin - 1 : (int64_t)big[i - 1];
    const int64_t cur = i == nb ? kmax + 1 : (int64_t)big[i];
    if (cur == prev) continue;
    int64_t k = cur - prev > kGapFill ? cur : prev + 1;
    if (k != prev + 1) *long_gap = 1;
    const int64_t hi = cur < kmax + 1 ? cur : kmax + 1;
    for (k = k < kmin ? kmin : k; k <= hi; ++k) first[k - kmin] = (I)i;
  }
}

template <typename K, typename I>
__global__ __launch_bounds__(kBlock) void dense_fill_kernel(const K* __restrict__ big, int64_t nb, int64_t kmin,
                                                           int64_t span, I sentinel, I* __restrict__ first) {
  for (int64_t k = blockIdx.x * (int64_t)blockDim.x + threadIdx.x; k <= span; k += (int64_t)gridDim.x * blockDim.x) {
    if (first[k] != sentinel) continue;
    const int64_t key = kmin + k;
    int64_t a = 0, b = nb;
    while (a < b) {
      const int64_t m = (a + b) >> 1;
      if ((int64_t)big[m] < key) a = m + 1;
      else b = m;
    }
    first[k] = (I)a;
  }
}

template <typename K, typename I>
__global__ __launch_bounds__(kBlock) void dense_ranges_kernel(const I* __restrict__ first, int64_t kmin, int64_t kmax,
                                                             const K* __restrict__ q,
                                                             const uint8_t* __restrict__ qvalid, int64_t nq,
                                                             int64_t* __restrict__ lo_out,
                                                             int64_t* __restrict__ cnt_out) {
  for (int64_t i = blockIdx.x * (int64_t)blockDim.x + threadIdx.x; i < nq; i += (int64_t)gridDim.x * blockDim.x) {
    const int64_t k = (int64_t)q[i];
    int64_t lo = 0, c = 0;
    if ((!qvalid || qvalid[i]) && k >= kmin && k <= kmax) {
      lo = (int64_t)first[k - kmin];
      c = (int64_t)first[k - kmin + 1] - lo;
    }
    lo_out[i] = lo;
    cnt_out[i] = c;
  }
}

}

void dense_index_build(const void* big, bool key64, int64_t nb, int64_t kmin, int64_t kmax, void* first, bool first64,
                       int32_t* long_gap, hipStream_t stream) {
  const dim3 b(kBlock);
  dispatch(wide{key64}, wide{first64}, [&](auto k, auto i) {
    using K = type_of<decltype(k)>;
    using I = type_of<decltype(i)>;
    if (!long_gap) {
      const int64_t span = kmax - kmin + 1;
      const dim3 g(grid_for(span + 1, kBlock, 1 << 16));
      launch("dense_index_build", dense_fill_kernel<K, I>, g, b, 0, stream, as<K>(big), nb, kmin, span, (I)-1,
             as<I>(first));
    } else {
      const dim3 g(grid_for(nb + 1, kBlock, 1 << 16));
      launch("dense_index_build", dense_index_kernel<K, I>, g, b, 0, stream, as<K>(big), nb, kmin, kmax, as<I>(first),
             long_gap);
    }
  });
}

void dense_ranges(const void* first, bool first64, int64_t kmin, int64_t kmax, const void* q, bool key64,
                  const uint8_t* qvalid, int64_t nq, int64_t* lo, int64_t* cnt, hipStream_t stream) {
  if (nq <= 0) return;
  const dim3 g(grid_for(nq, kBlock, 1 << 16)), b(kBlock);
  dispatch(wide{key64}, wide{first64}, [&](auto k, auto i) {
    using K = type_of<decltype(k)>;
    using I = type_of<decltype(i)>;
    launch("dense_ranges", dense_ranges_kernel<K, I>, g, b, 0, stream, as<I>(first), kmin, kmax, as<K>(q), qvalid, nq,
           lo, cnt);
  });
}

}
}

namespace igloo {
namespace kern {
namespace {
template <typename K2>
__global__ __launch_bounds__(kBlock) void sorted_exists_kernel(const K2* __restrict__ big2,
                                                              const K2* __restrict__ small2,
                                                              const int64_t* __restrict__ lo,
                                                              const int64_t* __restrict__ cnt, int64_t ns, int op,
                                                              const uint8_t* __restrict__ mask,
                                                              uint8_t* __restrict__ hit) {
  for (int64_t i = blockIdx.x * (int64_t)blockDim.x + threadIdx.x; i < ns; i += (int64_t)gridDim.x * blockDim.x) {
    const int64_t l = lo[i], c = cnt[i];
    const K2 v = op == 6 ? K2{} : small2[i];
    bool any = false;
    for (int64_t k = 0; k < c && !any; ++k) {
      if (mask && !mask[l + k]) continue;
      const K2 b = op == 6 ? K2{} : big2[l + k];
      switch (op) {
        case 0: any = b == v; break;
        case 1: any = b != v; break;
        case 2: any = b < v; break;
        case 3: any = b <= v; break;
        case 4: any = b > v; break;
        case 5: any = b >= v; break;
        default: any = true; break;
      }
    }
    hit[i] = any;
  }
}
}

void sorted_exists(const void* big2, const void* small2, bool key64, const int64_t* lo, const int64_t* cnt,
                   int64_t ns, int op, const uint8_t* mask, uint8_t* hit, hipStream_t stream) {
  if (ns <= 0) return;
  const dim3 g(grid_for(ns, kBlock, 1 << 16)), b(kBlock);
  dispatch(wide{key64}, [&](auto k) {
    using K2 = type_of<decltype(k)>;
    launch("sorted_exists", sorted_exists_kernel<K2>, g, b, 0, stream, as<K2>(big2), as<K2>(small2), lo, cnt, ns, op,
           mask, hit);
  });
}
}
}

namespace igloo {
namespace kern {
namespace {

template <typename K>
__global__ __launch_bounds__(kBlock) void unique_search_kernel(const K* __restrict__ big, int64_t nb,
                                                              const K* __restrict__ q,
                                                              const uint8_t* __restrict__ qvalid, int64_t nq,
                                                              uint8_t* __restrict__ hit, int32_t* __restrict__ pos,
                                                              const K* __restrict__ fence, int64_t nf) {
  for (int64_t i = blockIdx.x * (int64_t)blockDim.x + threadIdx.x; i < nq; i += (int64_t)gridDim.x * blockDim.x) {
    if (qvalid && !qvalid[i]) {
      hit[i] = 0;
      pos[i] = 0;
      continue;
    }
    const K key = q[i];
    int64_t a = 0, b = nb;
    if (fence) {
      int64_t fa = 0, fb = nf;
      while (fa < fb) {
        const int64_t m = (fa + fb) >> 1;
        if (fence[m] < key) fa = m + 1;
        else fb = m;
      }
      a = fa > 0 ? (fa - 1) * kFence : 0;
      b = fa * kFence < nb ? fa * kFence : nb;
    }
    while (a < b) {
      const int64_t m = (a + b) >> 1;
      if (big[m] < key) a = m + 1;
      else b = m;
    }
    const bool h = a < nb && big[a] == key;
    hit[i] = h ? 1 : 0;
    pos[i] = h ? (int32_t)a : 0;
  }
}

template <typename K, typename I>
__global__ __launch_bounds__(kBlock) void unique_dense_kernel(const I* __restrict__ first, int64_t kmin, int64_t kmax,
                                                             const K* __restrict__ q,
                                                             const uint8_t* __restrict__ qvalid, int64_t nq,
                                                             uint8_t* __restrict__ hit, int32_t* __restrict__ pos) {
  for (int64_t i = blockIdx.x * (int64_t)blockDim.x + threadIdx.x; i < nq; i += (int64_t)gridDim.x * blockDim.x) {
    const int64_t k = (int64_t)q[i];
    int64_t lo = 0;
    bool h = false;
    if ((!qvalid || qvalid[i]) && k >= kmin && k <= kmax) {
      lo = (int64_t)first[k - kmin];
      h = (int64_t)first[k - kmin + 1] > lo;
    }
    hit[i] = h ? 1 : 0;
    pos[i] = h ? (int32_t)lo : 0;
  }
}

}

void unique_lookup(const void* big, bool key64, int64_t nb, const void* first, bool first64, int64_t kmin,
                   int64_t kmax, const void* q, const uint8_t* qvalid, int64_t nq, uint8_t* hit, int32_t* pos,
                   const void* fence, int64_t nf, hipStream_t stream) {
  if (nq <= 0) return;
  const dim3 g(grid_for(nq, kBlock, 1 << 16)), b(kBlock);
  dispatch(wide{key64}, wide{first64}, [&](auto k, auto i) {
    using K = type_of<decltype(k)>;
    using I = type_of<decltype(i)>;
    if (first) {
      launch("unique_lookup", unique_dense_kernel<K, I>, g, b, 0, stream, as<I>(first), kmin, kmax, as<K>(q), qvalid,
             nq, hit, pos);
    } else {
      launch("unique_lookup", unique_search_kernel<K>, g, b, 0, stream, as<K>(big), nb, as<K>(q), qvalid, nq, hit, pos,
             as<K>(fence), nf);
    }
  });
}

}
}
```

csrc/kernels/scan.hip:

```cpp
#include "common.h"
#include "kernels.h"
#include "launch.h"

namespace igloo {
namespace kern {

namespace {

constexpr int kItems = 8;
constexpr int kTile = kBlock * kItems;

template <typename T>
__global__ __launch_bounds__(kBlock) void tile_sum_kernel(const T* __restrict__ in, int64_t n,
                                                         int64_t* __restrict__ sums) {
  __shared__ int64_t red[kWavesPerBlock];
  int64_t base = (int64_t)blockIdx.x * kTile + threadIdx.x;
  int64_t s = 0;
#pragma unroll
  for (int j = 0; j < kItems; ++j) {
    int64_t i = base + (int64_t)j * kBlock;
    if (i < n) s += (int64_t)in[i];
  }
  s = wave_reduce_sum(s);
  if (lane_id() == 0) red[threadIdx.x / kWave] = s;
  __syncthreads();
  if (threadIdx.x == 0) {
    int64_t t = 0;
    for (int w = 0; w < kWavesPerBlock; ++w) t += red[w];
    sums[blockIdx.x] = t;
  }
}

template <typename T>
__global__ __launch_bounds__(kBlock) void tile_scan_kernel(const T* __restrict__ in, int64_t n,
                                                          const int64_t* __restrict__ tile_off,
                                                          int64_t* __restrict__ out) {
  __shared__ int64_t scratch[kWavesPerBlock + 1];
  static_assert(kItems == 8, "vector path assumes 8 items per lane");
  const int64_t base = (int64_t)blockIdx.x * kTile + (int64_t)threadIdx.x * kItems;
  const bool whole = base + kItems <= n && (((uintptr_t)(in + base)) & 15) == 0 &&
                     (((uintptr_t)(out + base)) & 15) == 0;
  int64_t v[kItems];
  if (whole) {
    if (sizeof(T) == 4) {
      const uint4 a = reinterpret_cast<const uint4*>(in + base)[0], b = reinterpret_cast<const uint4*>(in + base)[1];
      const uint32_t w[8] = {a.x, a.y, a.z, a.w, b.x, b.y, b.z, b.w};
#pragma unroll
      for (int j = 0; j < kItems; ++j) v[j] = (int64_t)(int32_t)w[j];
    } else {
#pragma unroll
      for (int q = 0; q < kItems / 2; ++q) {
        const longlong2 x = reinterpret_cast<const longlong2*>(in + base)[q];
        v[2 * q] = x.x;
        v[2 * q + 1] = x.y;
      }
    }
  } else {
#pragma unroll
    for (int j = 0; j < kItems; ++j) v[j] = base + j < n ? (int64_t)in[base + j] : 0;
  }
  int64_t s = 0;
#pragma unroll
  for (int j = 0; j < kItems; ++j) s += v[j];
  int64_t total;
  int64_t run = tile_off[blockIdx.x] + block_exclusive_scan(s, scratch, &total);
  if (whole) {
#pragma unroll
    for (int q = 0; q < kItems / 2; ++q) {
      longlong2 x;
      x.x = run;
      run += v[2 * q];
      x.y = run;
      run += v[2 * q + 1];
      reinterpret_cast<longlong2*>(out + base)[q] = x;
    }
  } else {
#pragma unroll
    for (int j = 0; j < kItems; ++j) {
      if (base + j < n) out[base + j] = run;
      run += v[j];
    }
  }
}

constexpr int kSmallItems = 32;
constexpr int64_t kSmall = (int64_t)kBlock * kSmallItems;

template <typename T>
__global__ __launch_bounds__(kBlock) void small_scan_kernel(const T* __restrict__ in, int64_t n,
                                                           int64_t* __restrict__ out, int64_t* __restrict__ total) {
  __shared__ int64_t scratch[kWavesPerBlock + 1];
  const int64_t base = (int64_t)threadIdx.x * kSmallItems;
  int64_t v[kSmallItems];
#pragma unroll
  for (int j = 0; j < kSmallItems; ++j) v[j] = base + j < n ? (int64_t)in[base + j] : 0;
  int64_t s = 0;
#pragma unroll
  for (int j = 0; j < kSmallItems; ++j) s += v[j];
  int64_t tot;
  int64_t run = block_exclusive_scan(s, scratch, &tot);
#pragma unroll
  for (int j = 0; j < kSmallItems; ++j) {
    if (base + j < n) out[base + j] = run;
    run += v[j];
  }
  if (threadIdx.x == 0 && total) *total = tot;
}

template <typename T>
void exclusive_scan_impl(const T* in, int64_t n, int64_t* out, int64_t* tile_ws, int64_t* total,
                         hipStream_t stream) {
  int64_t tiles = (n + kTile - 1) / kTile;
  if (tiles == 0) {
    IGLOO_HIP_CHECK(hipMemsetAsync(total, 0, sizeof(int64_t), stream));
    return;
  }
  if (n <= kSmall) {
    launch("scan.small", small_scan_kernel<T>, dim3(1), dim3(kBlock), 0, stream, in, n, out, total);
    return;
  }
  launch("scan.tile_sum", tile_sum_kernel<T>, dim3((unsigned)tiles), dim3(kBlock), 0, stream, in, n, tile_ws);
  scan_counts(tile_ws, tiles, total, stream);
  launch("scan.tile_scan", tile_scan_kernel<T>, dim3((unsigned)tiles), dim3(kBlock), 0, stream, in, n, tile_ws, out);
}

}

int64_t scan_workspace_tiles(int64_t n) { return (n + kTile - 1) / kTile; }

void exclusive_scan(const void* in, bool in64, int64_t n, int64_t* out, int64_t* tile_ws, int64_t* total,
                    hipStream_t stream) {
  dispatch(wide{in64}, [&](auto t) {
    exclusive_scan_impl(as<type_of<decltype(t)>>(in), n, out, tile_ws, total, stream);
  });
}

}
}
```

igloo_amd/ops/hashing.py:

```python
from __future__ import annotations

from ..utils import switches as _sw
import contextvars
from typing import List, Optional, Sequence, Tuple

import torch

from ..utils import tags
from .gather import origin as _origin
from ._lib import capturing, check_not_capturing, is_gpu, launch, native, ptr, stream, to_host_f64s, to_host_int, to_host_ints, unlogged
from .select import exclusive_scan, mask_to_indices

EMPTY_KEY = -(2**63)
INT32_MAX = 2**31 - 1
BLOOM_MAX_KEYS = 4 << 20
BLOOM_MIN_RATIO = 4
EXACT_BITMAP = True
EXACT_BITMAP_MAX_SPAN = 1 << 25
DIRECT_JOIN_MAX_SPAN = 1 << 26

TABLE_BYTES_LIMIT: "contextvars.ContextVar[Optional[int]]" = contextvars.ContextVar("igloo_table_bytes", default=None)
PROBE_SELECT = True


def _next_pow2(x: int) -> int:
    p = 1
    while p < x:
        p <<= 1
    return p


def column_stats(keys: torch.Tensor, valid: Optional[torch.Tensor] = None) -> Tuple[Optional[Tuple[int, int]], bool]:
    if valid is None:
        hit = tags.STATS.get(keys)
        if hit is not None:
            return hit
    n = keys.numel()
    if not is_gpu(keys) or keys.dtype not in (torch.int32, torch.int64):
        k = keys if valid is None else keys[valid]
        if k.numel() == 0:
            return None, True
        mn, mx = torch.aminmax(k)
        srt = True if k.numel() < 2 else bool((k[1:] >= k[:-1]).all().item())
        return (int(mn.item()), int(mx.item())), srt
    N = launch("column_stats")
    buf = torch.empty(N.STATS_SLOTS, dtype=torch.int64, device=keys.device)
    N.column_stats(ptr(keys.contiguous()), keys.dtype == torch.int64,
                   ptr(valid.contiguous() if valid is not None else None), n, ptr(buf), stream(keys))
    out = buf[:3]
    if valid is None and tags.RESIDENT.get(keys, False):
        with unlogged():
            mn, mx, bad = to_host_ints(out)
    else:
        mn, mx, bad = to_host_ints(out)
    res = ((mn, mx) if mn <= mx else None), (bad == 0 and valid is None)
    if valid is None:
        if tags.STATS.set(keys, res) and tags.RESIDENT.get(keys, False):
            tags.SORTED.set(keys, res[1])
    return res


def key_range(keys: torch.Tensor, valid: Optional[torch.Tensor] = None) -> Optional[Tuple[int, int]]:
    return column_stats(keys, valid)[0]


BOUND_TRUST_ROWS = 1 << 20


CHECK_KEY_TAGS = _sw.debug("key_tags")


def _check_bound(keys: torch.Tensor, b: Tuple[int, int]) -> Tuple[int, int]:
    if CHECK_KEY_TAGS and keys.numel() and not capturing():
        lo, hi = to_host_ints(torch.stack([keys.min().to(torch.int64), keys.max().to(torch.int64)]))
        if lo < b[0] or hi > b[1]:
            raise AssertionError(f"key_bound {b} does not hold the keys' range [{lo}, {hi}]")
    return b


def key_bound(keys: torch.Tensor) -> Optional[Tuple[int, int]]:
    b = tags.BOUND.get(keys)
    if b is not None:
        return _check_bound(keys, b)
    o = _origin(keys)
    if o is None or o.dtype != keys.dtype or o.dim() != 1:
        return None
    st = tags.STATS.get(o)
    if st is None:
        if capturing():
            return None
        st = column_stats(o)
    return _check_bound(keys, st[0]) if st[0] is not None else None


UNIQUE_CHECK_MAX_ROWS = 1 << 27


def _check_unique(keys: torch.Tensor, why: str) -> bool:
    if CHECK_KEY_TAGS and keys.numel() > 1 and not capturing():
        n = keys.numel()
        u = torch.unique(keys.to(torch.int64)).numel()
        if u != n:
            raise AssertionError(f"key_unique() trusted {why} on {n} keys with {n - u} duplicates")
    return True


def key_unique(keys: torch.Tensor) -> bool:
    if tags.DISTINCT.get(keys, False):
        return _check_unique(keys, "a distinct tag")
    o = keys if tags.RESIDENT.get(keys, False) else tags.base_column(keys)
    if o is None or not tags.RESIDENT.get(o, False):
        return False
    u = tags.UNIQUE.get(o)
    if u is None:
        if capturing() or not is_gpu(o) or o.dim() != 1:
            return False
        if TABLE_BYTES_LIMIT.get() is not None or (o.numel() > UNIQUE_CHECK_MAX_ROWS and not is_sorted(o)):
            return False
        with unlogged():
            n = o.numel()
            if n < 2:
                u = True
            elif column_stats(o)[1]:
                u = to_host_int((o[1:] == o[:-1]).any().to(torch.int64)) == 0
            else:
                u = group_ids(o)[1] == n
        if not tags.UNIQUE.set(o, u):
            return False
    return u and _check_unique(keys, "the resident base column's uniqueness" if o is not keys else
                               "a resident column's uniqueness")


def _keys_ok(k: torch.Tensor) -> torch.Tensor:
    assert k.dim() == 1 and k.dtype in (torch.int32, torch.int64), f"join keys must be int32/int64, got {k.dtype}"
    return k.contiguous()


def _key_column(keys: torch.Tensor, valid: Optional[torch.Tensor] = None):
    return native().KeyColumn(ptr(keys), keys.dtype == torch.int64, ptr(valid), keys.numel())


class JoinTable:

    def __init__(self, keys: torch.Tensor, valid: Optional[torch.Tensor] = None, defer_unique: bool = False):
        keys = _keys_ok(keys)
        self.n = n = keys.numel()
        self._dups = None
        self.device = keys.device
        self.gpu = is_gpu(keys)
        self.valid = valid
        rng = None
        if valid is None and self.gpu:
            bnd = key_bound(keys)
            if bnd is not None and (self._direct_for(bnd[1] - bnd[0] + 1, n) or n < BOUND_TRUST_ROWS):
                rng = bnd
        if rng is None:
            rng = key_range(keys, valid)
        self.empty = rng is None
        if self.empty:
            self.unique = True
            return
        self.kmin, kmax = rng
        span = kmax - self.kmin + 1
        self.direct = self._direct_for(span, n)
        if not self.gpu:
            rows = None if valid is None else torch.nonzero(valid).reshape(-1)
            k = keys if rows is None else keys.index_select(0, rows)
            sk, order = torch.sort(k.to(torch.int64), stable=True)
            if rows is not None:
                order = rows.index_select(0, order)
            self.sorted_keys, self.order = sk, order
            self.unique = bool((sk[1:] != sk[:-1]).all().item()) if sk.numel() > 1 else True
            return
        known_unique = valid is None and key_unique(keys)
        N = launch("join_build")
        self.cap = span if self.direct else _next_pow2(2 * n)
        self.slots = self.cap if self.direct else self.cap + 1
        self.bits, self.bmask, self._fold = None, 0, None
        if self.direct and EXACT_BITMAP and span <= EXACT_BITMAP_MAX_SPAN:
            self.bits = torch.empty((span + 31) // 32, dtype=torch.int32, device=self.device)
            self.bmask = 1 << 63
        elif n <= BLOOM_MAX_KEYS:
            nbits = min(max(_next_pow2(8 * n), 1 << 15), 1 << 25)
            self.bits = torch.empty(nbits // 32, dtype=torch.int32, device=self.device)
            self.bmask = nbits - 1
        self.rid = torch.int32 if n < INT32_MAX else torch.int64
        self.rid64 = self.rid == torch.int64
        self.thead = torch.empty(self.slots, dtype=self.rid, device=self.device)
        self.tkeys = torch.empty(1 if self.direct else self.slots, dtype=torch.int64, device=self.device)
        dups = torch.empty(1, dtype=torch.int64, device=self.device)
        st = stream(keys)
        N.join_table_init(ptr(self.thead), self.rid64, self.slots, 0 if self.direct else ptr(self.tkeys),
                          ptr(self.bits), 0 if self.bits is None else self.bits.numel(), ptr(dups), st)
        self.cstart = self.crows = None
        self._set_ref()
        N.join_build(self._ref, _key_column(keys, valid), ptr(dups), st)
        if known_unique and CHECK_KEY_TAGS and not capturing():
            if to_host_int(dups) != 0:
                raise AssertionError("key_unique() trusted a key tag on keys that hold duplicates")
        self._csr_src = (keys, valid)
        if known_unique:
            self._unique = True
        elif defer_unique:
            self._unique, self._dups = None, dups
        else:
            self._set_unique(to_host_int(dups) == 0)

    @property
    def unique(self) -> bool:
        if self._unique is None:
            self._set_unique(to_host_int(self._dups) == 0)
        return self._unique

    @unique.setter
    def unique(self, v: bool) -> None:
        self._unique = v

    def _set_unique(self, u: bool) -> None:
        self._unique, self._dups = u, None
        if not u:
            keys, valid = self._csr_src
            col = _key_column(keys, valid)
            st = stream(keys)
            cnt = torch.zeros(self.slots + 1, dtype=self.rid, device=self.device)
            launch("join_csr_count").join_csr_count(self._ref, col, ptr(cnt), st)
            self.cstart = torch.zeros(self.slots + 1, dtype=self.rid, device=self.device)
            torch.cumsum(cnt[:-1], 0, dtype=self.rid, out=self.cstart[1:])
            self.crows = torch.empty(self.n, dtype=self.rid, device=self.device)
            self._set_ref()
            launch("join_csr_scatter").join_csr_scatter(self._ref, col, ptr(cnt), st)

    def _set_ref(self) -> None:
        self._ref = native().JoinTableRef(
            tkeys=ptr(self.tkeys), thead=ptr(self.thead), cstart=ptr(self.cstart), crows=ptr(self.crows),
            rid64=self.rid64, cap=self.cap, kmin=self.kmin, direct=self.direct, bits=ptr(self.bits),
            bmask=self.bmask, fold=ptr(self._fold), n_build=self.n)

    @staticmethod
    def _direct_for(span: int, n: int) -> bool:
        lim = TABLE_BYTES_LIMIT.get()
        wide_ok = span <= DIRECT_JOIN_MAX_SPAN and (lim is None or 12 * span <= lim)
        return span < 2**31 - 1 and (span <= 4 * n + 4096 or wide_ok)

    def probe_first(self, pkeys: torch.Tensor, pvalid: Optional[torch.Tensor] = None,
                    build_matched: Optional[torch.Tensor] = None) -> torch.Tensor:
        self.unique
        pkeys = _keys_ok(pkeys)
        m = pkeys.numel()
        if self.empty or m == 0:
            return torch.full((m,), -1, dtype=torch.int32, device=pkeys.device)
        if not self.gpu:
            cnt, lo = self._cpu_ranges(pkeys, pvalid)
            first = torch.where(cnt > 0, self.order.index_select(0, lo.clamp(max=max(self.order.numel() - 1, 0))),
                                torch.full_like(lo, -1)).to(torch.int32)
            if build_matched is not None:
                self._cpu_mark(cnt, lo, build_matched)
            return first
        first = torch.empty(m, dtype=self.rid, device=pkeys.device)
        launch("join_probe").join_probe(self._ref, _key_column(pkeys, pvalid), self._use_filter(m), 0, ptr(first),
                                        ptr(build_matched), stream(pkeys))
        return first

    def probe_select(self, pkeys: torch.Tensor, pvalid: Optional[torch.Tensor] = None, negate: bool = False,
                     want_build: bool = True) -> Tuple[torch.Tensor, Optional[torch.Tensor]]:
        pkeys = _keys_ok(pkeys)
        m = pkeys.numel()
        dev = pkeys.device
        if not self.gpu or self.empty or m == 0 or not PROBE_SELECT:
            first = self.probe_first(pkeys, pvalid)
            if not self.unique and want_build and not negate:
                return None
            sel = mask_to_indices(first < 0 if negate else first >= 0)
            return sel, (first.index_select(0, sel.long()) if want_build and not negate else None)
        N = launch("probe_hits")
        st = stream(pkeys)
        col = _key_column(pkeys, pvalid)
        tiles = N.probe_hit_tiles(m)
        words = torch.empty(tiles * 128, dtype=torch.int64, device=dev)
        tcount = torch.empty(tiles, dtype=torch.int64, device=dev)
        use_filter = self._use_filter(m)
        if use_filter:
            self._fold_scratch(m, st)
        N.probe_hits(self._ref, col, use_filter, negate, ptr(words), ptr(tcount), st)
        if self._unique is None:
            toff, tdev = exclusive_scan(tcount, host_total=False)
            dups, total = to_host_ints(torch.cat([self._dups.reshape(-1)[:1], tdev.reshape(-1)[:1]]))
            self._set_unique(dups == 0)
            if dups and want_build and not negate:
                return None
        else:
            toff, total = exclusive_scan(tcount)
        it = torch.int32 if m < INT32_MAX else torch.int64
        pidx = torch.empty(total, dtype=it, device=dev)
        bidx = torch.empty(total, dtype=self.rid, device=dev) if want_build and not negate else None
        if total:
            N.probe_write(self._ref, col, ptr(words), ptr(toff), ptr(pidx), it == torch.int64, ptr(bidx),
                          pidx.numel(), st)
        tags.INCR.set(pidx, True)
        return pidx, bidx

    def probe_pairs(self, pkeys: torch.Tensor, pvalid: Optional[torch.Tensor] = None,
                    build_matched: Optional[torch.Tensor] = None) -> Tuple[torch.Tensor, torch.Tensor, torch.Tensor]:
        self.unique
        pkeys = _keys_ok(pkeys)
        m = pkeys.numel()
        dev = pkeys.device
        if self.empty or m == 0:
            z = torch.zeros(0, dtype=torch.int32, device=dev)
            return z, z, torch.zeros(m, dtype=torch.int32, device=dev)
        if not self.gpu:
            cnt, lo = self._cpu_ranges(pkeys, pvalid)
            if build_matched is not None:
                self._cpu_mark(cnt, lo, build_matched)
            total = int(cnt.sum().item())
            pidx = torch.repeat_interleave(torch.arange(m), cnt)
            starts = torch.cumsum(cnt, 0) - cnt
            within = torch.arange(total) - starts.index_select(0, pidx)
            bpos = lo.index_select(0, pidx) + within
            bidx = self.order.index_select(0, bpos)
            return pidx.to(torch.int32), bidx.to(torch.int32), cnt.to(torch.int32)
        if m >= INT32_MAX:
            raise ValueError(f"probe_pairs: {m} probe rows exceed int32 probe ids; split the probe side")
        N = launch("join_probe")
        s = stream(pkeys)
        counts = torch.empty(m, dtype=torch.int32, device=dev)
        col = _key_column(pkeys, pvalid)
        use_filter = self._use_filter(m)
        N.join_probe(self._ref, col, use_filter, ptr(counts), 0, ptr(build_matched), s)
        offsets, total = exclusive_scan(counts)
        pidx = torch.empty(total, dtype=torch.int32, device=dev)
        bidx = torch.empty(total, dtype=self.rid, device=dev)
        if total:
            launch("join_expand")
            N.join_expand(self._ref, col, use_filter, ptr(offsets), ptr(pidx), ptr(bidx), pidx.numel(), s)
        return pidx, bidx, counts

    def _use_filter(self, m: int) -> bool:
        return self.bits is not None and m >= BLOOM_MIN_RATIO * self.n

    def _bloom(self, m: int) -> Tuple[int, int]:
        return (ptr(self.bits), self.bmask) if self._use_filter(m) else (0, 0)

    def _fold_scratch(self, m: int, st: int) -> None:
        N = native()
        if self._fold is None and self.direct and self.bmask >> 63 and N.probe_fold_needed(m, self.cap):
            self._fold = torch.empty(N.kFoldWords, dtype=torch.int32, device=self.device)
            N.probe_fold_build(ptr(self.bits), self.cap, ptr(self._fold), st)
            self._set_ref()

    def _cpu_ranges(self, pkeys, pvalid):
        pk = pkeys.to(torch.int64)
        lo = torch.searchsorted(self.sorted_keys, pk, right=False)
        hi = torch.searchsorted(self.sorted_keys, pk, right=True)
        cnt = hi - lo
        if pvalid is not None:
            cnt = torch.where(pvalid, cnt, torch.zeros_like(cnt))
        return cnt, lo

    def _cpu_mark(self, cnt, lo, build_matched):
        total = int(cnt.sum().item())
        if total == 0:
            return
        pidx = torch.repeat_interleave(torch.arange(cnt.numel()), cnt)
        starts = torch.cumsum(cnt, 0) - cnt
        bpos = lo.index_select(0, pidx) + torch.arange(total) - starts.index_select(0, pidx)
        build_matched.index_fill_(0, self.order.index_select(0, bpos).long(), True)


SORTED_CHECK_ROWS = 1 << 20

def is_sorted(keys: torch.Tensor) -> bool:
    hit = tags.SORTED.get(keys)
    if hit is not None:
        if hit and CHECK_KEY_TAGS and not capturing() and not tags.RESIDENT.get(keys, False) \
                and keys.numel() > 1 and keys.is_cuda:
            if to_host_int((keys[1:] < keys[:-1]).any().to(torch.int64)):
                raise AssertionError("an inferred sorted tag does not hold")
        return hit
    base = tags.base_column(keys)
    if base is not None and is_sorted(base):
        return True
    r = keys.numel() < 2 or column_stats(keys)[1]
    tags.SORTED.set(keys, r)
    return r


DENSE_INDEX = True
DENSE_INDEX_MIN_QUERIES = 1 << 20
DENSE_INDEX_MAX_SPAN_RATIO = 4


def dense_index(big: torch.Tensor, build: bool = True, queries: Optional[int] = None):
    hit = tags.DENSE.get(big)
    resident = tags.RESIDENT.get(big, False) or tags.INDEX_KEYS.get(big, False)
    if hit or (hit is False and (queries is None or resident)):
        return hit or None
    if resident:
        if queries is None or queries < DENSE_RESIDENT_MIN_QUERIES:
            return None
        with unlogged():
            return _dense_index_build(big, None, resident=True)
    if not build:
        return None
    rng = tags.RANGE.get(big)
    if hit is False and rng is not None and rng[1] - rng[0] + 1 > _dense_limit(big.numel(), queries):
        return None
    return _dense_index_build(big, queries)


DENSE_RESIDENT_MIN_QUERIES = 4096
DENSE_RESIDENT_MAX_ENTRIES = 1 << 30


def _dense_limit(nb: int, queries: Optional[int], resident: bool = False) -> int:
    if resident:
        return max(DENSE_INDEX_MAX_SPAN_RATIO * nb, DENSE_RESIDENT_MAX_ENTRIES) + 4096
    return DENSE_INDEX_MAX_SPAN_RATIO * min(nb, queries if queries is not None else nb) + 4096


def _dense_index_build(big: torch.Tensor, queries: Optional[int], resident: bool = False):
    nb = big.numel()
    idx = False
    if nb:
        rng = tags.RANGE.get(big)
        if rng is None:
            rng = tuple(to_host_ints(torch.stack([big[0].to(torch.int64), big[-1].to(torch.int64)])))
            tags.RANGE.set(big, rng)
        kmin, kmax = rng
        span = kmax - kmin + 1
        if span <= _dense_limit(nb, queries, resident):
            it = torch.int64 if nb >= INT32_MAX else torch.int32
            first = torch.empty(span + 1, dtype=it, device=big.device)
            gap = torch.zeros(1, dtype=torch.int32, device=big.device)
            N = launch("dense_index_build")
            st = stream(big)
            N.dense_index_build(ptr(big), big.dtype == torch.int64, nb, kmin, kmax, ptr(first),
                                it == torch.int64, ptr(gap), st)
            if to_host_int(gap):
                first.fill_(-1)
                N.dense_index_build(ptr(big), big.dtype == torch.int64, nb, kmin, kmax, ptr(first),
                                    it == torch.int64, ptr(gap), st)
                N.dense_index_build(ptr(big), big.dtype == torch.int64, nb, kmin, kmax, ptr(first),
                                    it == torch.int64, 0, st)
            idx = (kmin, kmax, first)
    tags.DENSE.set(big, idx)
    return idx or None


def sorted_ranges(big: torch.Tensor, q: torch.Tensor, qvalid: Optional[torch.Tensor] = None
                  ) -> Tuple[torch.Tensor, torch.Tensor]:
    big = _keys_ok(big)
    q = q.to(big.dtype).contiguous()
    nq = q.numel()
    if not is_gpu(big):
        lo = torch.searchsorted(big, q)
        cnt = torch.searchsorted(big, q, right=True) - lo
        if qvalid is not None:
            cnt = torch.where(qvalid, cnt, torch.zeros_like(cnt))
        return lo, cnt
    lo = torch.empty(nq, dtype=torch.int64, device=big.device)
    cnt = torch.empty(nq, dtype=torch.int64, device=big.device)
    idx = dense_index(big, build=nq >= DENSE_INDEX_MIN_QUERIES, queries=nq) if DENSE_INDEX else None
    if idx:
        kmin, kmax, first = idx
        launch("dense_ranges").dense_ranges(ptr(first), first.dtype == torch.int64, kmin, kmax, ptr(q),
                                            q.dtype == torch.int64,
                                            ptr(qvalid.contiguous() if qvalid is not None else None), nq, ptr(lo),
                                            ptr(cnt), stream(big))
        return lo, cnt
    fence = search_fence(big) if SEARCH_FENCE else None
    launch("sorted_ranges").sorted_ranges(ptr(big), big.dtype == torch.int64, big.numel(), ptr(q),
                                          ptr(qvalid.contiguous() if qvalid is not None else None), nq, ptr(lo),
                                          ptr(cnt), ptr(fence), 0 if fence is None else fence.numel(), stream(big))
    return lo, cnt


def unique_lookup(big: torch.Tensor, q: torch.Tensor, qvalid: Optional[torch.Tensor] = None
                  ) -> Optional[Tuple[torch.Tensor, torch.Tensor]]:
    big = _keys_ok(big)
    nb = big.numel()
    if nb >= 2**31 - 1:
        return None
    q = q.to(big.dtype).contiguous()
    nq = q.numel()
    if not is_gpu(big):
        lo = torch.searchsorted(big, q)
        hit = lo < nb
        if nb:
            hit &= big[lo.clamp(max=nb - 1)] == q
        if qvalid is not None:
            hit &= qvalid
        return hit, torch.where(hit, lo, torch.zeros_like(lo)).to(torch.int32)
    hit = torch.empty(nq, dtype=torch.bool, device=big.device)
    pos = torch.empty(nq, dtype=torch.int32, device=big.device)
    qv = ptr(qvalid.contiguous()) if qvalid is not None else 0
    idx = dense_index(big, build=nq >= DENSE_INDEX_MIN_QUERIES, queries=nq) if DENSE_INDEX else None
    N = launch("unique_lookup")
    if idx:
        kmin, kmax, first = idx
        N.unique_lookup(0, big.dtype == torch.int64, nb, ptr(first), first.dtype == torch.int64, kmin, kmax, ptr(q),
                        qv, nq, ptr(hit), ptr(pos), 0, 0, stream(big))
    else:
        fence = search_fence(big) if SEARCH_FENCE else None
        N.unique_lookup(ptr(big), big.dtype == torch.int64, nb, 0, False, 0, 0, ptr(q), qv, nq, ptr(hit), ptr(pos),
                        ptr(fence), 0 if fence is None else fence.numel(), stream(big))
    return hit, pos


SEARCH_FENCE = True
SEARCH_FENCE_MIN_ROWS = 1 << 22


def search_fence(big: torch.Tensor) -> Optional[torch.Tensor]:
    if big.numel() < SEARCH_FENCE_MIN_ROWS or not tags.RESIDENT.get(big, False):
        return None
    hit = tags.FENCE.get(big)
    if hit is None:
        check_not_capturing("search fence of a resident column")
        hit = big[::native().SEARCH_FENCE].contiguous()
        if not tags.FENCE.set(big, hit):
            return None
    return hit


def perm_index(keys: torch.Tensor) -> Tuple[torch.Tensor, torch.Tensor]:
    hit = tags.PERM.get(keys)
    if hit is not None:
        return hit
    from .sort import perm_sort_int
    with unlogged():
        out = perm_sort_int(keys)
    if tags.SORTED.set(out[0], True) and tags.INDEX_KEYS.set(out[0], True):
        tags.PERM.set(keys, out)
    return out


def expand_ranges(lo: torch.Tensor, cnt: torch.Tensor, big_n: int, scanned=None) -> Tuple[torch.Tensor, torch.Tensor]:
    ns = lo.numel()
    dev = lo.device
    off, total = scanned if scanned is not None else exclusive_scan(cnt)
    it = torch.int32 if max(total, big_n, ns) < INT32_MAX else torch.int64
    if not is_gpu(lo):
        sidx = torch.repeat_interleave(torch.arange(ns, dtype=it), cnt, output_size=total)
        bidx = (lo.index_select(0, sidx.long()) - off.index_select(0, sidx.long())
                + torch.arange(total, dtype=torch.int64)).to(it)
        return sidx, bidx
    sidx = torch.empty(total, dtype=it, device=dev)
    bidx = torch.empty(total, dtype=it, device=dev)
    if total:
        launch("expand_ranges").expand_ranges(ptr(off), ptr(lo.contiguous()), ns, total, ptr(sidx), ptr(bidx),
                                              it == torch.int64, stream(lo))
    return sidx, bidx


def sorted_match_pairs(big1: torch.Tensor, big2: torch.Tensor, small1: torch.Tensor, small2: torch.Tensor,
                       identity_ok: bool = False) -> Tuple[Optional[torch.Tensor], torch.Tensor]:
    lo, cnt = sorted_ranges(big1, small1)
    ns = small1.numel()
    big2 = _keys_ok(big2)
    small2 = small2.to(big2.dtype).contiguous()
    if not is_gpu(big1):
        s, b = expand_ranges(lo, cnt, big1.numel())
        keep = big2.index_select(0, b.long()) == small2.index_select(0, s.long())
        return s[keep], b[keep]
    N = launch("sorted_match")
    st = stream(big1)
    counts = torch.empty(max(ns, 1), dtype=torch.int32, device=big1.device)
    k64 = big2.dtype == torch.int64
    first = torch.empty(ns, dtype=torch.int32, device=big1.device) \
        if identity_ok and ns and max(big1.numel(), ns) < INT32_MAX else None
    N.sorted_match(ptr(big2), ptr(small2), k64, ptr(lo), ptr(cnt), ns, ptr(counts), 0, 0, 0, False, 0, ptr(first), st)
    if first is not None:
        c = counts[:ns]
        total, odd = to_host_ints(torch.stack([c.sum(), (c != 1).sum()]))
        if odd == 0:
            return None, first
        off, _ = exclusive_scan(c, host_total=False)
    else:
        off, total = exclusive_scan(counts[:ns])
    it = torch.int32 if max(total, big1.numel(), ns) < INT32_MAX else torch.int64
    sidx = torch.empty(total, dtype=it, device=big1.device)
    bidx = torch.empty(total, dtype=it, device=big1.device)
    if total:
        N.sorted_match(ptr(big2), ptr(small2), k64, ptr(lo), ptr(cnt), ns, 0, ptr(off), ptr(sidx), ptr(bidx),
                       it == torch.int64, total, 0, st)
    return sidx, bidx


def masked_expand(lo: torch.Tensor, cnt: torch.Tensor, mask: torch.Tensor, big_n: int
                  ) -> Tuple[torch.Tensor, torch.Tensor]:
    ns = lo.numel()
    if not is_gpu(lo):
        s, b = expand_ranges(lo, cnt, big_n)
        keep = mask.index_select(0, b.long())
        return s[keep], b[keep]
    N = launch("sorted_masked")
    st = stream(lo)
    mk = mask.contiguous().view(torch.uint8)
    counts = torch.empty(max(ns, 1), dtype=torch.int32, device=lo.device)
    N.sorted_masked(ptr(mk), ptr(lo), ptr(cnt), ns, ptr(counts), 0, 0, 0, False, 0, st)
    off, total = exclusive_scan(counts[:ns])
    it = torch.int32 if max(total, big_n, ns) < INT32_MAX else torch.int64
    sidx = torch.empty(total, dtype=it, device=lo.device)
    bidx = torch.empty(total, dtype=it, device=lo.device)
    if total:
        N.sorted_masked(ptr(mk), ptr(lo), ptr(cnt), ns, 0, ptr(off), ptr(sidx), ptr(bidx), it == torch.int64, total,
                        st)
    return sidx, bidx


EXISTS_OPS = {"=": 0, "<>": 1, "<": 2, "<=": 3, ">": 4, ">=": 5, "any": 6}


def sorted_exists(big2: Optional[torch.Tensor], small2: Optional[torch.Tensor], lo: torch.Tensor, cnt: torch.Tensor,
                  op: str, mask: Optional[torch.Tensor] = None) -> torch.Tensor:
    ns = lo.numel()
    if op == "any":
        big2 = small2 = None
        dt = torch.int32
    else:
        dt = torch.int64 if torch.int64 in (big2.dtype, small2.dtype) else torch.int32
        big2, small2 = big2.to(dt).contiguous(), small2.to(dt).contiguous()
    if not is_gpu(lo):
        nb = mask.numel() if mask is not None else big2.numel()
        s, b = expand_ranges(lo, cnt, nb)
        if op == "any":
            ok = torch.ones(s.numel(), dtype=torch.bool)
        else:
            bv, sv = big2.index_select(0, b.long()), small2.index_select(0, s.long())
            ok = {"=": bv == sv, "<>": bv != sv, "<": bv < sv, "<=": bv <= sv, ">": bv > sv, ">=": bv >= sv}[op]
        if mask is not None:
            ok = ok & mask.index_select(0, b.long())
        hit = torch.zeros(ns, dtype=torch.bool)
        hit.index_fill_(0, s.long()[ok], True)
        return hit
    hit = torch.empty(ns, dtype=torch.bool, device=lo.device)
    mk = mask.contiguous().view(torch.uint8) if mask is not None else None
    launch("sorted_exists").sorted_exists(ptr(big2), ptr(small2), dt == torch.int64, ptr(lo), ptr(cnt), ns,
                                          EXISTS_OPS[op], ptr(mk), ptr(hit), stream(lo))
    return hit


def group_ids_ex(keys: torch.Tensor) -> Tuple[torch.Tensor, int, torch.Tensor, bool]:
    keys = _keys_ok(keys)
    n = keys.numel()
    if n >= SORTED_CHECK_ROWS and is_gpu(keys):
        if is_sorted(keys):
            bound = torch.empty(n, dtype=torch.bool, device=keys.device)
            launch("run_bounds").run_bounds(ptr(keys), keys.dtype == torch.int64, n, ptr(bound), stream(keys))
            starts = mask_to_indices(bound)
            g = starts.numel()
            gid = torch.empty(n, dtype=torch.int32, device=keys.device)
            launch("fill_runs").fill_runs(ptr(starts), starts.dtype == torch.int64, g, n, ptr(gid), stream(keys))
            tags.BOUND.set(gid, (0, max(g - 1, 0)))
            return gid, g, starts.to(torch.int32), True
    gid, g, rep = group_ids(keys)
    return gid, g, rep, False


def _group_table(keys: torch.Tensor, n: int) -> Tuple[int, bool, int]:
    bnd = key_bound(keys)
    if bnd is not None and (bnd[1] - bnd[0] + 1 <= 2 * n + 65536 or n < BOUND_TRUST_ROWS):
        kmin, kmax = bnd
    elif tags.HASHED.get(keys, False) and n > 1:
        kmin, kmax = 0, 2**62
    else:
        kmin, kmax = key_range(keys)
    span = kmax - kmin + 1
    direct = span <= 2 * n + 65536 and span < 2**31 - 1
    return kmin, direct, span if direct else _next_pow2(2 * n)


def _group_slots(direct: bool, cap: int) -> int:
    return cap if direct else cap + 1


def _group_build(keys: torch.Tensor, n: int):
    kmin, direct, cap = _group_table(keys, n)
    dev = keys.device
    nslots = _group_slots(direct, cap)
    trow = torch.full((nslots,), INT32_MAX, dtype=torch.int32, device=dev)
    tkeys = (torch.empty(1, dtype=torch.int64, device=dev) if direct
             else torch.full((nslots,), EMPTY_KEY, dtype=torch.int64, device=dev))
    launch("groupby").groupby_build(ptr(keys), keys.dtype == torch.int64, n, ptr(tkeys), ptr(trow), cap, kmin,
                                    direct, stream(keys))
    return kmin, direct, cap, nslots, tkeys, trow


def group_ids(keys: torch.Tensor) -> Tuple[torch.Tensor, int, torch.Tensor]:
    keys = _keys_ok(keys)
    n = keys.numel()
    dev = keys.device
    if n == 0:
        z = torch.zeros(0, dtype=torch.int32, device=dev)
        return z, 0, z
    if not is_gpu(keys):
        uniq, inv = torch.unique(keys, sorted=True, return_inverse=True)
        g = uniq.numel()
        rep = torch.full((g,), n, dtype=torch.int64).scatter_reduce(0, inv, torch.arange(n), reduce="amin")
        return inv.to(torch.int32), g, rep.to(torch.int32)
    kmin, direct, cap, nslots, tkeys, trow = _group_build(keys, n)
    N = native()
    s = stream(keys)
    occ = torch.empty(nslots, dtype=torch.bool, device=dev)
    gid_of_slot = torch.empty(nslots, dtype=torch.int32, device=dev)
    N.groupby_occupied(ptr(trow), nslots, ptr(occ), ptr(gid_of_slot), s)
    slots = mask_to_indices(occ)
    g = slots.numel()
    rep = torch.empty(g, dtype=torch.int32, device=dev)
    N.groupby_assign(ptr(slots), slots.dtype == torch.int64, g, nslots, ptr(trow), ptr(gid_of_slot), ptr(rep), s)
    gid = torch.empty(n, dtype=torch.int32, device=dev)
    N.groupby_lookup(ptr(keys), keys.dtype == torch.int64, n, ptr(tkeys), ptr(gid_of_slot), cap, kmin, direct, ptr(gid), s)
    if not direct and g > 1:
        from .gather import gather_tensor
        first = rep.clamp(max=n - 1).long()
        mark = torch.zeros(n, dtype=torch.bool, device=dev)
        mark.index_fill_(0, first, True)
        order = mask_to_indices(mark, total=g)
        newpos = torch.zeros(n, dtype=torch.int32, device=dev)
        newpos.index_copy_(0, order.long(), torch.arange(order.numel(), dtype=torch.int32, device=dev))
        remap = newpos.index_select(0, first)
        gid = gather_tensor(remap, gid)
        rep = order.to(torch.int32)
    tags.BOUND.set(gid, (0, max(g - 1, 0)))
    return gid, g, rep


def first_rows_mask(keys: torch.Tensor) -> torch.Tensor:
    keys = _keys_ok(keys)
    n = keys.numel()
    dev = keys.device
    if n == 0 or not is_gpu(keys):
        mark = torch.zeros(n, dtype=torch.bool, device=dev)
        if n:
            _, _, rep = group_ids(keys)
            mark[rep.long()] = True
        return mark
    _, _, _, nslots, _, trow = _group_build(keys, n)
    mark = torch.zeros(n, dtype=torch.bool, device=dev)
    launch("mark_slot_rows").mark_slot_rows(ptr(trow), nslots, n, ptr(mark), stream(keys))
    return mark


HLL_BITS = 12
HLL_M = 1 << HLL_BITS


def hll_sketch(keys: torch.Tensor, valid: Optional[torch.Tensor] = None) -> Optional[torch.Tensor]:
    src = keys
    if valid is None:
        hit = tags.HLL.get(src)
        if hit is not None:
            return hit
    if valid is None and tags.RESIDENT.get(src, False):
        check_not_capturing("sketch of a resident column")
    keys = _keys_ok(keys)
    n = keys.numel()
    if not is_gpu(keys):
        return None
    regs = torch.zeros(HLL_M, dtype=torch.uint8, device=keys.device)
    if n == 0:
        return regs
    N = launch("hll_sketch")
    ws = torch.empty(N.hll_blocks(n) * HLL_M, dtype=torch.uint8, device=keys.device)
    N.hll_sketch(ptr(keys), keys.dtype == torch.int64, ptr(valid), n, ptr(ws), ptr(regs), stream(keys))
    if valid is None:
        tags.HLL.set(src, regs)
    return regs


def hll_terms(regs: torch.Tensor) -> torch.Tensor:
    r = regs.to(torch.float64)
    return torch.stack([torch.pow(2.0, -r).sum(-1), (regs == 0).sum(-1).to(torch.float64)], -1)


def hll_estimate(regs: torch.Tensor) -> float:
    z, zeros = to_host_f64s(hll_terms(regs))
    return hll_from_terms(z, int(zeros))


def hll_from_terms(z: float, zeros: int) -> float:
    m = float(HLL_M)
    alpha = 0.7213 / (1.0 + 1.079 / m)
    e = alpha * m * m / z
    if e <= 2.5 * m and zeros > 0:
        import math
        e = m * math.log(m / zeros)
    return e


def ndv(keys: torch.Tensor, valid: Optional[torch.Tensor] = None) -> int:
    if keys.numel() == 0:
        return 0
    if is_gpu(keys):
        return max(1, int(round(hll_estimate(hll_sketch(keys, valid)))))
    k = keys if valid is None else keys[valid]
    return int(torch.unique(k).numel())


def pack_keys(cols: Sequence[torch.Tensor]) -> torch.Tensor:
    assert cols
    if len(cols) == 1:
        c = cols[0]
        return c if c.dtype in (torch.int32, torch.int64) else c.to(torch.int64)
    ranges = _bounded_ranges(cols)
    bits = [max(1, int(hi - lo).bit_length()) for lo, hi in ranges]
    if sum(bits) <= 62:
        return _pack_bits(cols, ranges, bits)
    acc = cols[0].to(torch.int64)
    for c in cols[1:]:
        g1, n1, _ = group_ids(acc)
        g2, n2, _ = group_ids(c.to(torch.int64) if c.dtype != torch.int64 else c)
        acc = g1.to(torch.int64) * max(n2, 1) + g2.to(torch.int64)
    return acc


def pack_keys_pair(left: Sequence[torch.Tensor], right: Sequence[torch.Tensor]) -> Tuple[torch.Tensor, torch.Tensor]:
    if len(left) == 1:
        return left[0], right[0]
    nl = left[0].numel()
    if is_gpu(left[0]) and len(left) <= MAX_PACK_BITS:
        both = _bounded_ranges(list(left) + list(right))
        rl, rr = both[:len(left)], both[len(left):]
        if right[0].numel() == 0:
            ranges = rl
        elif nl == 0:
            ranges = rr
        else:
            ranges = [(min(a[0], b[0]), max(a[1], b[1])) for a, b in zip(rl, rr)]
        bits = [max(1, int(hi - lo).bit_length()) for lo, hi in ranges]
        if sum(bits) <= 62:
            return _pack_bits(list(left), ranges, bits), _pack_bits(list(right), ranges, bits)
    both = [torch.cat([a.to(torch.int64), b.to(torch.int64)]) for a, b in zip(left, right)]
    packed = pack_keys(both)
    return packed[:nl], packed[nl:]


MAX_PACK_BITS = 8


def key_ranges(cols: Sequence[torch.Tensor]) -> List[Tuple[int, int]]:
    out: List[Optional[Tuple[int, int]]] = [None] * len(cols)
    todo = []
    for i, c in enumerate(cols):
        if c.numel() == 0:
            out[i] = (0, 0)
            continue
        hit = tags.STATS.get(c)
        if hit is not None and hit[0] is not None:
            out[i] = hit[0]
        elif is_gpu(c) and c.dtype in (torch.int32, torch.int64) and c.dim() == 1:
            todo.append(i)
        else:
            r = key_range(c)
            out[i] = r if r is not None else (0, 0)
    if todo:
        N = launch("column_stats")
        bufs = []
        for i in todo:
            c = cols[i].contiguous()
            buf = torch.empty(N.STATS_SLOTS, dtype=torch.int64, device=c.device)
            N.column_stats(ptr(c), c.dtype == torch.int64, 0, c.numel(), ptr(buf), stream(c))
            bufs.append(buf[:2])
        vals = to_host_ints(torch.cat(bufs))
        for j, i in enumerate(todo):
            lo, hi = vals[2 * j], vals[2 * j + 1]
            out[i] = (lo, hi) if lo <= hi else (0, 0)
    return out


def _bounded_ranges(cols: Sequence[torch.Tensor]) -> List[Tuple[int, int]]:
    out: List[Optional[Tuple[int, int]]] = [None] * len(cols)
    todo = []
    for i, c in enumerate(cols):
        b = key_bound(c) if is_gpu(c) and c.numel() else None
        if b is not None:
            out[i] = b
        else:
            todo.append(i)
    if todo:
        for i, r in zip(todo, key_ranges([cols[i] for i in todo])):
            out[i] = r
    return out


def _pack_bits(cols: Sequence[torch.Tensor], ranges, bits) -> torch.Tensor:
    n = cols[0].numel()
    if not is_gpu(cols[0]) or len(cols) > MAX_PACK_BITS or any(c.dtype not in (torch.int32, torch.int64)
                                                                for c in cols):
        out = None
        for c, (lo, _), b in zip(cols, ranges, bits):
            v = c.to(torch.int64) - lo
            out = v if out is None else (out << b) | v
        return out
    cs = [c.contiguous() for c in cols]
    out = torch.empty(n, dtype=torch.int64, device=cs[0].device)
    shifts = [0] + list(bits[1:])
    launch("pack_bits").pack_bits([ptr(c) for c in cs], [c.dtype == torch.int64 for c in cs],
                                  [int(lo) for lo, _ in ranges], shifts, n, ptr(out), stream(out))
    return out
```

Baseline: 0.06320.

## Narrow join range buffers to int32 and chunk the exclusive scan into two passes

Sorted-range lookups now emit lo/cnt as int32 when the build side fits in 32 bits, and every range consumer kernel is templated on the range type. This halves the range buffer traffic and allocation size for joins. The exclusive scan is also reorganised so each block handles a chunk of tiles with a running carry. That drops the separate tile-count scan launch. The cost is more template instantiations and width-conversion checks on the Python side.

```diff
diff --git a/csrc/bindings.cpp b/csrc/bindings.cpp
--- a/csrc/bindings.cpp
+++ b/csrc/bindings.cpp
@@ -633,10 +633,10 @@
                             S(s));
   });
   m.def("dense_ranges", [](uintptr_t first, bool first64, int64_t kmin, int64_t kmax, uintptr_t q, bool key64,
-                           uintptr_t qvalid, int64_t nq, uintptr_t lo, uintptr_t cnt, uintptr_t s) {
+                           uintptr_t qvalid, int64_t nq, uintptr_t lo, uintptr_t cnt, bool range64, uintptr_t s) {
     if (nq > 0 && (!first || !q || !lo || !cnt)) throw std::runtime_error("dense_ranges: null buffer");
     kern::dense_ranges(P<const void>(first), first64, kmin, kmax, P<const void>(q), key64, P<const uint8_t>(qvalid), nq,
-                       P<int64_t>(lo), P<int64_t>(cnt), S(s));
+                       P<void>(lo), P<void>(cnt), range64, S(s));
   });
   m.def("unique_lookup", [](uintptr_t big, bool key64, int64_t nb, uintptr_t first, bool first64, int64_t kmin,
                             int64_t kmax, uintptr_t q, uintptr_t qvalid, int64_t nq, uintptr_t hit, uintptr_t pos,
@@ -647,28 +647,28 @@
                         P<const uint8_t>(qvalid), nq, P<uint8_t>(hit), P<int32_t>(pos), P<const void>(fence), nf,
                         S(s));
   });
-  m.def("sorted_exists", [](uintptr_t big2, uintptr_t small2, bool key64, uintptr_t lo, uintptr_t cnt, int64_t ns,
-                            int op, uintptr_t mask, uintptr_t hit, uintptr_t s) {
+  m.def("sorted_exists", [](uintptr_t big2, uintptr_t small2, bool key64, uintptr_t lo, uintptr_t cnt, bool range64,
+                            int64_t ns, int op, uintptr_t mask, uintptr_t hit, uintptr_t s) {
     if (op < 0 || op > 6 || (op == 6 && !mask) || (ns > 0 && (!lo || !cnt || !hit || (op < 6 && (!big2 || !small2)))))
       throw std::runtime_error("sorted_exists: bad arguments");
-    kern::sorted_exists(P<const void>(big2), P<const void>(small2), key64, P<const int64_t>(lo), P<const int64_t>(cnt),
-                        ns, op, P<const uint8_t>(mask), P<uint8_t>(hit), S(s));
-  });
-  m.def("sorted_match", [](uintptr_t big2, uintptr_t small2, bool key64, uintptr_t lo, uintptr_t cnt, int64_t ns,
-                           uintptr_t counts, uintptr_t offsets, uintptr_t sidx, uintptr_t bidx, bool out64,
+    kern::sorted_exists(P<const void>(big2), P<const void>(small2), key64, P<const void>(lo), P<const void>(cnt),
+                        range64, ns, op, P<const uint8_t>(mask), P<uint8_t>(hit), S(s));
+  });
+  m.def("sorted_match", [](uintptr_t big2, uintptr_t small2, bool key64, uintptr_t lo, uintptr_t cnt, bool range64,
+                           int64_t ns, uintptr_t counts, uintptr_t offsets, uintptr_t sidx, uintptr_t bidx, bool out64,
                            int64_t out_cap, uintptr_t first, uintptr_t s) {
     if (ns > 0 && (!big2 || !small2 || !lo || !cnt || (!offsets && !counts) || (offsets && (!sidx || !bidx))))
       throw std::runtime_error("sorted_match: null buffer");
-    kern::sorted_match(P<const void>(big2), P<const void>(small2), key64, P<const int64_t>(lo), P<const int64_t>(cnt),
-                       ns, P<int32_t>(counts), P<const int64_t>(offsets), P<void>(sidx), P<void>(bidx), out64,
+    kern::sorted_match(P<const void>(big2), P<const void>(small2), key64, P<const void>(lo), P<const void>(cnt),
+                       range64, ns, P<int32_t>(counts), P<const int64_t>(offsets), P<void>(sidx), P<void>(bidx), out64,
                        out_cap, P<int32_t>(first), S(s));
   });
-  m.def("sorted_masked", [](uintptr_t mask, uintptr_t lo, uintptr_t cnt, int64_t ns, uintptr_t counts,
+  m.def("sorted_masked", [](uintptr_t mask, uintptr_t lo, uintptr_t cnt, bool range64, int64_t ns, uintptr_t counts,
                             uintptr_t offsets, uintptr_t sidx, uintptr_t bidx, bool out64, int64_t out_cap,
                             uintptr_t s) {
     if (ns > 0 && (!mask || !lo || !cnt || (!offsets && !counts) || (offsets && (!sidx || !bidx))))
       throw std::runtime_error("sorted_masked: null buffer");
-    kern::sorted_masked(P<const uint8_t>(mask), P<const int64_t>(lo), P<const int64_t>(cnt), ns, P<int32_t>(counts),
+    kern::sorted_masked(P<const uint8_t>(mask), P<const void>(lo), P<const void>(cnt), range64, ns, P<int32_t>(counts),
                         P<const int64_t>(offsets), P<void>(sidx), P<void>(bidx), out64, out_cap, S(s));
   });
 
diff --git a/csrc/kernels/kernels.h b/csrc/kernels/kernels.h
--- a/csrc/kernels/kernels.h
+++ b/csrc/kernels/kernels.h
@@ -445,22 +445,22 @@
 
 constexpr int64_t kFence = 256;
 void sorted_ranges(const void* big, bool key64, int64_t nb, const void* q, const uint8_t* qvalid, int64_t nq,
-                   int64_t* lo, int64_t* cnt, const void* fence, int64_t nf, hipStream_t stream);
-void expand_ranges(const int64_t* off, const int64_t* lo, int64_t ns, int64_t total, void* sidx, void* bidx,
-                   bool out64, hipStream_t stream);
+                   void* lo, void* cnt, bool range64, const void* fence, int64_t nf, hipStream_t stream);
+void expand_ranges(const int64_t* off, const void* lo, bool range64, int64_t ns, int64_t total, void* sidx,
+                   void* bidx, bool out64, hipStream_t stream);
 void dense_index_build(const void* big, bool key64, int64_t nb, int64_t kmin, int64_t kmax, void* first, bool first64,
                        int32_t* long_gap, hipStream_t stream);
 void dense_ranges(const void* first, bool first64, int64_t kmin, int64_t kmax, const void* q, bool key64,
-                  const uint8_t* qvalid, int64_t nq, int64_t* lo, int64_t* cnt, hipStream_t stream);
+                  const uint8_t* qvalid, int64_t nq, void* lo, void* cnt, bool range64, hipStream_t stream);
 void unique_lookup(const void* big, bool key64, int64_t nb, const void* first, bool first64, int64_t kmin,
                    int64_t kmax, const void* q, const uint8_t* qvalid, int64_t nq, uint8_t* hit, int32_t* pos,
                    const void* fence, int64_t nf, hipStream_t stream);
-void sorted_exists(const void* big2, const void* small2, bool key64, const int64_t* lo, const int64_t* cnt,
+void sorted_exists(const void* big2, const void* small2, bool key64, const void* lo, const void* cnt, bool range64,
                    int64_t ns, int op, const uint8_t* mask, uint8_t* hit, hipStream_t stream);
-void sorted_match(const void* big2, const void* small2, bool key64, const int64_t* lo, const int64_t* cnt,
+void sorted_match(const void* big2, const void* small2, bool key64, const void* lo, const void* cnt, bool range64,
                   int64_t ns, int32_t* counts, const int64_t* offsets, void* sidx, void* bidx, bool out64,
                   int64_t out_cap, int32_t* first, hipStream_t stream);
-void sorted_masked(const uint8_t* mask, const int64_t* lo, const int64_t* cnt, int64_t ns, int32_t* counts,
+void sorted_masked(const uint8_t* mask, const void* lo, const void* cnt, bool range64, int64_t ns, int32_t* counts,
                    const int64_t* offsets, void* sidx, void* bidx, bool out64, int64_t out_cap, hipStream_t stream);
 
 enum PqPhys : int { PQ_PHYS_BOOLEAN = 0, PQ_PHYS_INT32 = 1, PQ_PHYS_INT64 = 2, PQ_PHYS_INT96 = 3, PQ_PHYS_FLOAT = 4,
diff --git a/csrc/kernels/ranges.hip b/csrc/kernels/ranges.hip
--- a/csrc/kernels/ranges.hip
+++ b/csrc/kernels/ranges.hip
@@ -11,12 +11,12 @@
 constexpr int kExpTile = kBlock * kExpItems;
 constexpr int kScanRun = 16;
 
-template <typename K>
+template <typename K, typename R>
 __global__ __launch_bounds__(kBlock) void sorted_ranges_kernel(const K* __restrict__ big, int64_t nb,
                                                               const K* __restrict__ q,
                                                               const uint8_t* __restrict__ qvalid, int64_t nq,
-                                                              int64_t* __restrict__ lo_out,
-                                                              int64_t* __restrict__ cnt_out,
+                                                              R* __restrict__ lo_out,
+                                                              R* __restrict__ cnt_out,
                                                               const K* __restrict__ fence, int64_t nf) {
   for (int64_t i = blockIdx.x * (int64_t)blockDim.x + threadIdx.x; i < nq; i += (int64_t)gridDim.x * blockDim.x) {
     if (qvalid && !qvalid[i]) {
@@ -56,8 +56,8 @@
       }
       e = a2;
     }
-    lo_out[i] = a;
-    cnt_out[i] = e - a;
+    lo_out[i] = (R)a;
+    cnt_out[i] = (R)(e - a);
   }
 }
 
@@ -71,9 +71,9 @@
   return a;
 }
 
-template <typename O>
+template <typename O, typename R>
 __global__ __launch_bounds__(kBlock) void expand_ranges_kernel(const int64_t* __restrict__ off,
-                                                              const int64_t* __restrict__ lo, int64_t ns,
+                                                              const R* __restrict__ lo, int64_t ns,
                                                               int64_t total, O* __restrict__ sidx,
                                                               O* __restrict__ bidx) {
   __shared__ int64_t soff[kExpTile + 1];
@@ -93,14 +93,14 @@
     const int64_t ta = t0 + (int64_t)threadIdx.x * kExpItems;
     if (ta < t1) {
       int64_t j = row_of(soff, nr, ta);
-      int64_t base = lo[r0 + j] - soff[j];
+      int64_t base = (int64_t)lo[r0 + j] - soff[j];
       O sv[kExpItems], bv[kExpItems];
 #pragma unroll
       for (int k = 0; k < kExpItems; ++k) {
         const int64_t t = ta + k;
         while (j + 1 < nr && soff[j + 1] <= t) {
           ++j;
-          base = lo[r0 + j] - soff[j];
+          base = (int64_t)lo[r0 + j] - soff[j];
         }
         sv[k] = (O)(r0 + j);
         bv[k] = (O)(base + t);
@@ -134,7 +134,7 @@
       if (t >= t1) break;
       const int64_t r = row_of(off, ns, t);
       sidx[t] = (O)r;
-      bidx[t] = (O)(lo[r] + (t - off[r]));
+      bidx[t] = (O)((int64_t)lo[r] + (t - off[r]));
     }
   }
 }
@@ -142,24 +142,26 @@
 }
 
 void sorted_ranges(const void* big, bool key64, int64_t nb, const void* q, const uint8_t* qvalid, int64_t nq,
-                   int64_t* lo, int64_t* cnt, const void* fence, int64_t nf, hipStream_t stream) {
+                   void* lo, void* cnt, bool range64, const void* fence, int64_t nf, hipStream_t stream) {
   if (nq <= 0) return;
   const unsigned grid = grid_for(nq, kBlock, 1 << 16);
-  dispatch(wide{key64}, [&](auto k) {
+  dispatch(wide{key64}, wide{range64}, [&](auto k, auto r) {
     using K = type_of<decltype(k)>;
-    launch("sorted_ranges", sorted_ranges_kernel<K>, dim3(grid), dim3(kBlock), 0, stream, as<K>(big), nb, as<K>(q),
-           qvalid, nq, lo, cnt, as<K>(fence), nf);
-  });
-}
-
-void expand_ranges(const int64_t* off, const int64_t* lo, int64_t ns, int64_t total, void* sidx, void* bidx,
-                   bool out64, hipStream_t stream) {
+    using R = type_of<decltype(r)>;
+    launch("sorted_ranges", sorted_ranges_kernel<K, R>, dim3(grid), dim3(kBlock), 0, stream, as<K>(big), nb, as<K>(q),
+           qvalid, nq, as<R>(lo), as<R>(cnt), as<K>(fence), nf);
+  });
+}
+
+void expand_ranges(const int64_t* off, const void* lo, bool range64, int64_t ns, int64_t total, void* sidx,
+                   void* bidx, bool out64, hipStream_t stream) {
   if (total <= 0 || ns <= 0) return;
   const unsigned grid = (unsigned)((total + kExpTile - 1) / kExpTile);
-  dispatch(wide{out64}, [&](auto o) {
+  dispatch(wide{out64}, wide{range64}, [&](auto o, auto r) {
     using O = type_of<decltype(o)>;
-    launch("expand_ranges", expand_ranges_kernel<O>, dim3(grid), dim3(kBlock), 0, stream, off, lo, ns, total,
-           as<O>(sidx), as<O>(bidx));
+    using R = type_of<decltype(r)>;
+    launch("expand_ranges", expand_ranges_kernel<O, R>, dim3(grid), dim3(kBlock), 0, stream, off, as<R>(lo), ns,
+           total, as<O>(sidx), as<O>(bidx));
   });
 }
 
@@ -170,18 +172,18 @@
 namespace kern {
 namespace {
 
-template <typename K2, typename O, bool WRITE, bool MASKED = false>
+template <typename K2, typename O, typename R, bool WRITE, bool MASKED = false>
 __global__ __launch_bounds__(kBlock) void sorted_match_kernel(const K2* __restrict__ big2,
                                                              const K2* __restrict__ small2,
-                                                             const int64_t* __restrict__ lo,
-                                                             const int64_t* __restrict__ cnt, int64_t ns,
+                                                             const R* __restrict__ lo,
+                                                             const R* __restrict__ cnt, int64_t ns,
                                                              int32_t* __restrict__ counts,
                                                              const int64_t* __restrict__ offsets,
                                                              O* __restrict__ sidx, O* __restrict__ bidx,
                                                              int64_t out_cap, O* __restrict__ first) {
   const uint8_t* __restrict__ mask = reinterpret_cast<const uint8_t*>(big2);
   for (int64_t i = blockIdx.x * (int64_t)blockDim.x + threadIdx.x; i < ns; i += (int64_t)gridDim.x * blockDim.x) {
-    const int64_t l = lo[i], c = cnt[i];
+    const int64_t l = (int64_t)lo[i], c = (int64_t)cnt[i];
     const K2 key = MASKED ? K2{} : small2[i];
     int64_t o = WRITE ? offsets[i] : 0;
     int32_t m = 0;
@@ -207,39 +209,42 @@
 }
 
 template <typename K2, bool MASKED>
-void launch_match(const char* what, const void* big2, const void* small2, const int64_t* lo, const int64_t* cnt,
-                  int64_t ns, int32_t* counts, const int64_t* offsets, void* sidx, void* bidx, bool out64,
-                  int64_t out_cap, int32_t* first, hipStream_t stream) {
+void launch_match(const char* what, const void* big2, const void* small2, const void* lo, const void* cnt,
+                  bool range64, int64_t ns, int32_t* counts, const int64_t* offsets, void* sidx, void* bidx,
+                  bool out64, int64_t out_cap, int32_t* first, hipStream_t stream) {
   const dim3 g(grid_for(ns, kBlock, 1 << 16)), b(kBlock);
-  if (!offsets) {
-    launch(what, sorted_match_kernel<K2, int32_t, false, MASKED>, g, b, 0, stream, as<K2>(big2), as<K2>(small2), lo,
-           cnt, ns, counts, nullptr, nullptr, nullptr, 0, first);
-    return;
-  }
-  dispatch(wide{out64}, [&](auto o) {
-    using O = type_of<decltype(o)>;
-    launch(what, sorted_match_kernel<K2, O, true, MASKED>, g, b, 0, stream, as<K2>(big2), as<K2>(small2), lo, cnt, ns,
-           nullptr, offsets, as<O>(sidx), as<O>(bidx), out_cap, nullptr);
-  });
-}
-
-}
-
-void sorted_match(const void* big2, const void* small2, bool key64, const int64_t* lo, const int64_t* cnt,
+  dispatch(wide{range64}, [&](auto r) {
+    using R = type_of<decltype(r)>;
+    if (!offsets) {
+      launch(what, sorted_match_kernel<K2, int32_t, R, false, MASKED>, g, b, 0, stream, as<K2>(big2), as<K2>(small2),
+             as<R>(lo), as<R>(cnt), ns, counts, nullptr, nullptr, nullptr, 0, first);
+      return;
+    }
+    dispatch(wide{out64}, [&](auto o) {
+      using O = type_of<decltype(o)>;
+      launch(what, sorted_match_kernel<K2, O, R, true, MASKED>, g, b, 0, stream, as<K2>(big2), as<K2>(small2),
+             as<R>(lo), as<R>(cnt), ns, nullptr, offsets, as<O>(sidx), as<O>(bidx), out_cap, nullptr);
+    });
+  });
+}
+
+}
+
+void sorted_match(const void* big2, const void* small2, bool key64, const void* lo, const void* cnt, bool range64,
                   int64_t ns, int32_t* counts, const int64_t* offsets, void* sidx, void* bidx, bool out64,
                   int64_t out_cap, int32_t* first, hipStream_t stream) {
   if (ns <= 0) return;
   dispatch(wide{key64}, [&](auto k) {
-    launch_match<type_of<decltype(k)>, false>("sorted_match", big2, small2, lo, cnt, ns, counts, offsets, sidx, bidx,
-                                              out64, out_cap, first, stream);
-  });
-}
-
-void sorted_masked(const uint8_t* mask, const int64_t* lo, const int64_t* cnt, int64_t ns, int32_t* counts,
+    launch_match<type_of<decltype(k)>, false>("sorted_match", big2, small2, lo, cnt, range64, ns, counts, offsets,
+                                              sidx, bidx, out64, out_cap, first, stream);
+  });
+}
+
+void sorted_masked(const uint8_t* mask, const void* lo, const void* cnt, bool range64, int64_t ns, int32_t* counts,
                    const int64_t* offsets, void* sidx, void* bidx, bool out64, int64_t out_cap, hipStream_t stream) {
   if (ns <= 0) return;
-  launch_match<int32_t, true>("sorted_masked", mask, nullptr, lo, cnt, ns, counts, offsets, sidx, bidx, out64, out_cap,
-                              nullptr, stream);
+  launch_match<int32_t, true>("sorted_masked", mask, nullptr, lo, cnt, range64, ns, counts, offsets, sidx, bidx, out64,
+                              out_cap, nullptr, stream);
 }
 
 }
@@ -282,12 +287,12 @@
   }
 }
 
-template <typename K, typename I>
+template <typename K, typename I, typename R>
 __global__ __launch_bounds__(kBlock) void dense_ranges_kernel(const I* __restrict__ first, int64_t kmin, int64_t kmax,
                                                              const K* __restrict__ q,
                                                              const uint8_t* __restrict__ qvalid, int64_t nq,
-                                                             int64_t* __restrict__ lo_out,
-                                                             int64_t* __restrict__ cnt_out) {
+                                                             R* __restrict__ lo_out,
+                                                             R* __restrict__ cnt_out) {
   for (int64_t i = blockIdx.x * (int64_t)blockDim.x + threadIdx.x; i < nq; i += (int64_t)gridDim.x * blockDim.x) {
     const int64_t k = (int64_t)q[i];
     int64_t lo = 0, c = 0;
@@ -295,8 +300,8 @@
       lo = (int64_t)first[k - kmin];
       c = (int64_t)first[k - kmin + 1] - lo;
     }
-    lo_out[i] = lo;
-    cnt_out[i] = c;
+    lo_out[i] = (R)lo;
+    cnt_out[i] = (R)c;
   }
 }
 
@@ -322,14 +327,15 @@
 }
 
 void dense_ranges(const void* first, bool first64, int64_t kmin, int64_t kmax, const void* q, bool key64,
-                  const uint8_t* qvalid, int64_t nq, int64_t* lo, int64_t* cnt, hipStream_t stream) {
+                  const uint8_t* qvalid, int64_t nq, void* lo, void* cnt, bool range64, hipStream_t stream) {
   if (nq <= 0) return;
   const dim3 g(grid_for(nq, kBlock, 1 << 16)), b(kBlock);
-  dispatch(wide{key64}, wide{first64}, [&](auto k, auto i) {
+  dispatch(wide{key64}, wide{first64}, wide{range64}, [&](auto k, auto i, auto r) {
     using K = type_of<decltype(k)>;
     using I = type_of<decltype(i)>;
-    launch("dense_ranges", dense_ranges_kernel<K, I>, g, b, 0, stream, as<I>(first), kmin, kmax, as<K>(q), qvalid, nq,
-           lo, cnt);
+    using R = type_of<decltype(r)>;
+    launch("dense_ranges", dense_ranges_kernel<K, I, R>, g, b, 0, stream, as<I>(first), kmin, kmax, as<K>(q), qvalid,
+           nq, as<R>(lo), as<R>(cnt));
   });
 }
 
@@ -339,15 +345,15 @@
 namespace igloo {
 namespace kern {
 namespace {
-template <typename K2>
+template <typename K2, typename R>
 __global__ __launch_bounds__(kBlock) void sorted_exists_kernel(const K2* __restrict__ big2,
                                                               const K2* __restrict__ small2,
-                                                              const int64_t* __restrict__ lo,
-                                                              const int64_t* __restrict__ cnt, int64_t ns, int op,
+                                                              const R* __restrict__ lo,
+                                                              const R* __restrict__ cnt, int64_t ns, int op,
                                                               const uint8_t* __restrict__ mask,
                                                               uint8_t* __restrict__ hit) {
   for (int64_t i = blockIdx.x * (int64_t)blockDim.x + threadIdx.x; i < ns; i += (int64_t)gridDim.x * blockDim.x) {
-    const int64_t l = lo[i], c = cnt[i];
+    const int64_t l = (int64_t)lo[i], c = (int64_t)cnt[i];
     const K2 v = op == 6 ? K2{} : small2[i];
     bool any = false;
     for (int64_t k = 0; k < c && !any; ++k) {
@@ -368,14 +374,15 @@
 }
 }
 
-void sorted_exists(const void* big2, const void* small2, bool key64, const int64_t* lo, const int64_t* cnt,
+void sorted_exists(const void* big2, const void* small2, bool key64, const void* lo, const void* cnt, bool range64,
                    int64_t ns, int op, const uint8_t* mask, uint8_t* hit, hipStream_t stream) {
   if (ns <= 0) return;
   const dim3 g(grid_for(ns, kBlock, 1 << 16)), b(kBlock);
-  dispatch(wide{key64}, [&](auto k) {
+  dispatch(wide{key64}, wide{range64}, [&](auto k, auto r) {
     using K2 = type_of<decltype(k)>;
-    launch("sorted_exists", sorted_exists_kernel<K2>, g, b, 0, stream, as<K2>(big2), as<K2>(small2), lo, cnt, ns, op,
-           mask, hit);
+    using R = type_of<decltype(r)>;
+    launch("sorted_exists", sorted_exists_kernel<K2, R>, g, b, 0, stream, as<K2>(big2), as<K2>(small2), as<R>(lo),
+           as<R>(cnt), ns, op, mask, hit);
   });
 }
 }
diff --git a/csrc/kernels/scan.hip b/csrc/kernels/scan.hip
--- a/csrc/kernels/scan.hip
+++ b/csrc/kernels/scan.hip
@@ -10,16 +10,33 @@
 constexpr int kItems = 8;
 constexpr int kTile = kBlock * kItems;
 
+constexpr int kMaxChunks = 2048;
+
+struct Chunking {
+  int64_t tiles, tiles_per_chunk, chunks;
+};
+
+Chunking chunking(int64_t n) {
+  Chunking c;
+  c.tiles = (n + kTile - 1) / kTile;
+  c.tiles_per_chunk = (c.tiles + kMaxChunks - 1) / kMaxChunks;
+  c.chunks = c.tiles_per_chunk ? (c.tiles + c.tiles_per_chunk - 1) / c.tiles_per_chunk : 0;
+  return c;
+}
+
 template <typename T>
-__global__ __launch_bounds__(kBlock) void tile_sum_kernel(const T* __restrict__ in, int64_t n,
+__global__ __launch_bounds__(kBlock) void tile_sum_kernel(const T* __restrict__ in, int64_t n, int64_t tiles_per_chunk,
                                                          int64_t* __restrict__ sums) {
   __shared__ int64_t red[kWavesPerBlock];
-  int64_t base = (int64_t)blockIdx.x * kTile + threadIdx.x;
+  const int64_t first = (int64_t)blockIdx.x * tiles_per_chunk * kTile;
+  const int64_t end = first + tiles_per_chunk * kTile < n ? first + tiles_per_chunk * kTile : n;
   int64_t s = 0;
+  for (int64_t base = first + threadIdx.x; base < end; base += kTile) {
 #pragma unroll
-  for (int j = 0; j < kItems; ++j) {
-    int64_t i = base + (int64_t)j * kBlock;
-    if (i < n) s += (int64_t)in[i];
+    for (int j = 0; j < kItems; ++j) {
+      int64_t i = base + (int64_t)j * kBlock;
+      if (i < end) s += (int64_t)in[i];
+    }
   }
   s = wave_reduce_sum(s);
   if (lane_id() == 0) red[threadIdx.x / kWave] = s;
@@ -33,54 +50,65 @@
 
 template <typename T>
 __global__ __launch_bounds__(kBlock) void tile_scan_kernel(const T* __restrict__ in, int64_t n,
-                                                          const int64_t* __restrict__ tile_off,
-                                                          int64_t* __restrict__ out) {
+                                                          int64_t tiles_per_chunk,
+                                                          const int64_t* __restrict__ sums,
+                                                          int64_t* __restrict__ out, int64_t* total) {
   __shared__ int64_t scratch[kWavesPerBlock + 1];
+  int64_t before = 0;
+  for (int j = threadIdx.x; j < (int)blockIdx.x; j += kBlock) before += sums[j];
+  int64_t carry;
+  block_exclusive_scan(before, scratch, &carry);
   static_assert(kItems == 8, "vector path assumes 8 items per lane");
-  const int64_t base = (int64_t)blockIdx.x * kTile + (int64_t)threadIdx.x * kItems;
-  const bool whole = base + kItems <= n && (((uintptr_t)(in + base)) & 15) == 0 &&
-                     (((uintptr_t)(out + base)) & 15) == 0;
-  int64_t v[kItems];
-  if (whole) {
-    if (sizeof(T) == 4) {
-      const uint4 a = reinterpret_cast<const uint4*>(in + base)[0], b = reinterpret_cast<const uint4*>(in + base)[1];
-      const uint32_t w[8] = {a.x, a.y, a.z, a.w, b.x, b.y, b.z, b.w};
+  const int64_t first = (int64_t)blockIdx.x * tiles_per_chunk * kTile;
+  const int64_t end = first + tiles_per_chunk * kTile < n ? first + tiles_per_chunk * kTile : n;
+  for (int64_t tile_base = first; tile_base < end; tile_base += kTile) {
+    const int64_t base = tile_base + (int64_t)threadIdx.x * kItems;
+    const bool whole = base + kItems <= n && (((uintptr_t)(in + base)) & 15) == 0 &&
+                       (((uintptr_t)(out + base)) & 15) == 0;
+    int64_t v[kItems];
+    if (whole) {
+      if (sizeof(T) == 4) {
+        const uint4 a = reinterpret_cast<const uint4*>(in + base)[0], b = reinterpret_cast<const uint4*>(in + base)[1];
+        const uint32_t w[8] = {a.x, a.y, a.z, a.w, b.x, b.y, b.z, b.w};
 #pragma unroll
-      for (int j = 0; j < kItems; ++j) v[j] = (int64_t)(int32_t)w[j];
+        for (int j = 0; j < kItems; ++j) v[j] = (int64_t)(int32_t)w[j];
+      } else {
+#pragma unroll
+        for (int q = 0; q < kItems / 2; ++q) {
+          const longlong2 x = reinterpret_cast<const longlong2*>(in + base)[q];
+          v[2 * q] = x.x;
+          v[2 * q + 1] = x.y;
+        }
+      }
     } else {
 #pragma unroll
+      for (int j = 0; j < kItems; ++j) v[j] = base + j < n ? (int64_t)in[base + j] : 0;
+    }
+    int64_t s = 0;
+#pragma unroll
+    for (int j = 0; j < kItems; ++j) s += v[j];
+    int64_t tile_total;
+    int64_t run = carry + block_exclusive_scan(s, scratch, &tile_total);
+    carry += tile_total;
+    if (whole) {
+#pragma unroll
       for (int q = 0; q < kItems / 2; ++q) {
-        const longlong2 x = reinterpret_cast<const longlong2*>(in + base)[q];
-        v[2 * q] = x.x;
-        v[2 * q + 1] = x.y;
+        longlong2 x;
+        x.x = run;
+        run += v[2 * q];
+        x.y = run;
+        run += v[2 * q + 1];
+        reinterpret_cast<longlong2*>(out + base)[q] = x;
+      }
+    } else {
+#pragma unroll
+      for (int j = 0; j < kItems; ++j) {
+        if (base + j < n) out[base + j] = run;
+        run += v[j];
       }
     }
-  } else {
-#pragma unroll
-    for (int j = 0; j < kItems; ++j) v[j] = base + j < n ? (int64_t)in[base + j] : 0;
   }
-  int64_t s = 0;
-#pragma unroll
-  for (int j = 0; j < kItems; ++j) s += v[j];
-  int64_t total;
-  int64_t run = tile_off[blockIdx.x] + block_exclusive_scan(s, scratch, &total);
-  if (whole) {
-#pragma unroll
-    for (int q = 0; q < kItems / 2; ++q) {
-      longlong2 x;
-      x.x = run;
-      run += v[2 * q];
-      x.y = run;
-      run += v[2 * q + 1];
-      reinterpret_cast<longlong2*>(out + base)[q] = x;
-    }
-  } else {
-#pragma unroll
-    for (int j = 0; j < kItems; ++j) {
-      if (base + j < n) out[base + j] = run;
-      run += v[j];
-    }
-  }
+  if (blockIdx.x == gridDim.x - 1 && threadIdx.x == 0 && total) *total = carry;
 }
 
 constexpr int kSmallItems = 32;
@@ -110,8 +138,8 @@
 template <typename T>
 void exclusive_scan_impl(const T* in, int64_t n, int64_t* out, int64_t* tile_ws, int64_t* total,
                          hipStream_t stream) {
-  int64_t tiles = (n + kTile - 1) / kTile;
-  if (tiles == 0) {
+  const Chunking c = chunking(n);
+  if (c.tiles == 0) {
     IGLOO_HIP_CHECK(hipMemsetAsync(total, 0, sizeof(int64_t), stream));
     return;
   }
@@ -119,14 +147,15 @@
     launch("scan.small", small_scan_kernel<T>, dim3(1), dim3(kBlock), 0, stream, in, n, out, total);
     return;
   }
-  launch("scan.tile_sum", tile_sum_kernel<T>, dim3((unsigned)tiles), dim3(kBlock), 0, stream, in, n, tile_ws);
-  scan_counts(tile_ws, tiles, total, stream);
-  launch("scan.tile_scan", tile_scan_kernel<T>, dim3((unsigned)tiles), dim3(kBlock), 0, stream, in, n, tile_ws, out);
+  launch("scan.tile_sum", tile_sum_kernel<T>, dim3((unsigned)c.chunks), dim3(kBlock), 0, stream, in, n,
+         c.tiles_per_chunk, tile_ws);
+  launch("scan.tile_scan", tile_scan_kernel<T>, dim3((unsigned)c.chunks), dim3(kBlock), 0, stream, in, n,
+         c.tiles_per_chunk, tile_ws, out, total);
 }
 
 }
 
-int64_t scan_workspace_tiles(int64_t n) { return (n + kTile - 1) / kTile; }
+int64_t scan_workspace_tiles(int64_t n) { return chunking(n).chunks; }
 
 void exclusive_scan(const void* in, bool in64, int64_t n, int64_t* out, int64_t* tile_ws, int64_t* total,
                     hipStream_t stream) {
diff --git a/igloo_amd/ops/hashing.py b/igloo_amd/ops/hashing.py
--- a/igloo_amd/ops/hashing.py
+++ b/igloo_amd/ops/hashing.py
@@ -458,21 +458,32 @@
         if qvalid is not None:
             cnt = torch.where(qvalid, cnt, torch.zeros_like(cnt))
         return lo, cnt
-    lo = torch.empty(nq, dtype=torch.int64, device=big.device)
-    cnt = torch.empty(nq, dtype=torch.int64, device=big.device)
+    rt = torch.int32 if RANGE32 and big.numel() < INT32_MAX else torch.int64
+    lo = torch.empty(nq, dtype=rt, device=big.device)
+    cnt = torch.empty(nq, dtype=rt, device=big.device)
     idx = dense_index(big, build=nq >= DENSE_INDEX_MIN_QUERIES, queries=nq) if DENSE_INDEX else None
     if idx:
         kmin, kmax, first = idx
         launch("dense_ranges").dense_ranges(ptr(first), first.dtype == torch.int64, kmin, kmax, ptr(q),
                                             q.dtype == torch.int64,
                                             ptr(qvalid.contiguous() if qvalid is not None else None), nq, ptr(lo),
-                                            ptr(cnt), stream(big))
+                                            ptr(cnt), rt == torch.int64, stream(big))
         return lo, cnt
     fence = search_fence(big) if SEARCH_FENCE else None
     launch("sorted_ranges").sorted_ranges(ptr(big), big.dtype == torch.int64, big.numel(), ptr(q),
                                           ptr(qvalid.contiguous() if qvalid is not None else None), nq, ptr(lo),
-                                          ptr(cnt), ptr(fence), 0 if fence is None else fence.numel(), stream(big))
+                                          ptr(cnt), rt == torch.int64, ptr(fence),
+                                          0 if fence is None else fence.numel(), stream(big))
     return lo, cnt
+
+
+RANGE32 = True
+
+
+def _range_pair(lo: torch.Tensor, cnt: torch.Tensor) -> Tuple[torch.Tensor, torch.Tensor, bool]:
+    if lo.dtype != cnt.dtype or lo.dtype not in (torch.int32, torch.int64):
+        lo, cnt = lo.to(torch.int64), cnt.to(torch.int64)
+    return lo.contiguous(), cnt.contiguous(), lo.dtype == torch.int64
 
 
 def unique_lookup(big: torch.Tensor, q: torch.Tensor, qvalid: Optional[torch.Tensor] = None
@@ -548,8 +559,9 @@
     sidx = torch.empty(total, dtype=it, device=dev)
     bidx = torch.empty(total, dtype=it, device=dev)
     if total:
-        launch("expand_ranges").expand_ranges(ptr(off), ptr(lo.contiguous()), ns, total, ptr(sidx), ptr(bidx),
-                                              it == torch.int64, stream(lo))
+        lo = lo.contiguous() if lo.dtype in (torch.int32, torch.int64) else lo.to(torch.int64)
+        launch("expand_ranges").expand_ranges(ptr(off), ptr(lo), lo.dtype == torch.int64, ns, total, ptr(sidx),
+                                              ptr(bidx), it == torch.int64, stream(lo))
     return sidx, bidx
 
 
@@ -565,11 +577,13 @@
         return s[keep], b[keep]
     N = launch("sorted_match")
     st = stream(big1)
+    lo, cnt, r64 = _range_pair(lo, cnt)
     counts = torch.empty(max(ns, 1), dtype=torch.int32, device=big1.device)
     k64 = big2.dtype == torch.int64
     first = torch.empty(ns, dtype=torch.int32, device=big1.device) \
         if identity_ok and ns and max(big1.numel(), ns) < INT32_MAX else None
-    N.sorted_match(ptr(big2), ptr(small2), k64, ptr(lo), ptr(cnt), ns, ptr(counts), 0, 0, 0, False, 0, ptr(first), st)
+    N.sorted_match(ptr(big2), ptr(small2), k64, ptr(lo), ptr(cnt), r64, ns, ptr(counts), 0, 0, 0, False, 0, ptr(first),
+                   st)
     if first is not None:
         c = counts[:ns]
         total, odd = to_host_ints(torch.stack([c.sum(), (c != 1).sum()]))
@@ -582,7 +596,7 @@
     sidx = torch.empty(total, dtype=it, device=big1.device)
     bidx = torch.empty(total, dtype=it, device=big1.device)
     if total:
-        N.sorted_match(ptr(big2), ptr(small2), k64, ptr(lo), ptr(cnt), ns, 0, ptr(off), ptr(sidx), ptr(bidx),
+        N.sorted_match(ptr(big2), ptr(small2), k64, ptr(lo), ptr(cnt), r64, ns, 0, ptr(off), ptr(sidx), ptr(bidx),
                        it == torch.int64, total, 0, st)
     return sidx, bidx
 
@@ -596,16 +610,17 @@
         return s[keep], b[keep]
     N = launch("sorted_masked")
     st = stream(lo)
+    lo, cnt, r64 = _range_pair(lo, cnt)
     mk = mask.contiguous().view(torch.uint8)
     counts = torch.empty(max(ns, 1), dtype=torch.int32, device=lo.device)
-    N.sorted_masked(ptr(mk), ptr(lo), ptr(cnt), ns, ptr(counts), 0, 0, 0, False, 0, st)
+    N.sorted_masked(ptr(mk), ptr(lo), ptr(cnt), r64, ns, ptr(counts), 0, 0, 0, False, 0, st)
     off, total = exclusive_scan(counts[:ns])
     it = torch.int32 if max(total, big_n, ns) < INT32_MAX else torch.int64
     sidx = torch.empty(total, dtype=it, device=lo.device)
     bidx = torch.empty(total, dtype=it, device=lo.device)
     if total:
-        N.sorted_masked(ptr(mk), ptr(lo), ptr(cnt), ns, 0, ptr(off), ptr(sidx), ptr(bidx), it == torch.int64, total,
-                        st)
+        N.sorted_masked(ptr(mk), ptr(lo), ptr(cnt), r64, ns, 0, ptr(off), ptr(sidx), ptr(bidx), it == torch.int64,
+                        total, st)
     return sidx, bidx
 
 
@@ -636,7 +651,8 @@
         return hit
     hit = torch.empty(ns, dtype=torch.bool, device=lo.device)
     mk = mask.contiguous().view(torch.uint8) if mask is not None else None
-    launch("sorted_exists").sorted_exists(ptr(big2), ptr(small2), dt == torch.int64, ptr(lo), ptr(cnt), ns,
+    lo, cnt, r64 = _range_pair(lo, cnt)
+    launch("sorted_exists").sorted_exists(ptr(big2), ptr(small2), dt == torch.int64, ptr(lo), ptr(cnt), r64, ns,
                                           EXISTS_OPS[op], ptr(mk), ptr(hit), stream(lo))
     return hit
 
```

Result: no change. 0.06330 (+0.2%).
